# guilherme439/NuZero

Hardware: AMD Instinct MI355X
Metric: self-play games/sec (+ MCTS node-expansions/sec), Tic-Tac-Toe 100 sims/move (higher is better)
Workload: dtype f32; 1 GPU; Tic_Tac_Toe, 100 sims/move, 4096 concurrent self-play games per GPU (65536 games per round), RecurrentNet(2,1,64,2) 2 recurrent iterations f32, tree statistics f64, legacy TTT search config; concurrent_games_per_gpu=4096, games_per_round_per_gpu=65536, sims_per_move=100, parallelism=1 GPU

## Files before the change

### include/nuzero_amd.h

```cpp
#ifndef NUZERO_AMD_H
#define NUZERO_AMD_H

#include <stdint.h>

#ifdef __cplusplus
extern "C" {
#endif

typedef struct nz_engine nz_engine;
typedef struct nz_rng nz_rng;
typedef int nz_status;

enum {
  NZ_OK = 0,
  NZ_ERR_ARG = 1,
  NZ_ERR_HIP = 2,
  NZ_ERR_STATE = 3,
  NZ_ERR_OVERFLOW = 4
};

enum { NZ_GAME_TIC_TAC_TOE = 0 };
enum { NZ_ACT_TANH = 0, NZ_ACT_RELU = 1 };
enum { NZ_ARCH_RECURRENT = 0, NZ_ARCH_RESNET = 1, NZ_ARCH_CONVNET = 2 };

typedef struct nz_search_cfg {
  int32_t mcts_simulations;
  int32_t keep_subtree;
  double pb_c_base;
  double pb_c_init;
  int32_t number_of_softmax_moves;
  int32_t training;
  double epsilon_softmax_exploration;
  double epsilon_random_exploration;
  double value_factor;
  double root_exploration_fraction;
  double root_dist_alpha;
  double root_dist_beta;
} nz_search_cfg;

typedef struct nz_game_desc {
  int32_t game;
  int32_t negate_player;
} nz_game_desc;

typedef struct nz_net_desc {
  int32_t in_channels;
  int32_t policy_channels;
  int32_t width;
  int32_t num_blocks;
  int32_t recall;
  int32_t value_activation;
  int32_t arch;
  int32_t kernel_size;
  int32_t hex;
} nz_net_desc;

typedef struct nz_dims {
  int32_t n_games;
  int32_t n_slots;
  int32_t num_actions;
  int32_t max_moves;
  int32_t state_channels, rows, cols;
  int32_t node_capacity;
} nz_dims;

const char* nz_version(void);
const char* nz_last_error(const nz_engine* e);

nz_status nz_engine_create(nz_engine** out, const nz_search_cfg* cfg, const nz_game_desc* game,
                           int32_t n_games, int32_t device);
nz_status nz_engine_create_ex(nz_engine** out, const nz_search_cfg* cfg, const nz_game_desc* game,
                              int32_t n_slots, int32_t n_games, int32_t device);
void nz_engine_destroy(nz_engine* e);
nz_status nz_engine_dims(const nz_engine* e, nz_dims* out);

nz_status nz_engine_set_weights(nz_engine* e, const nz_net_desc* net, const float* const* weights,
                                int32_t n_tensors, int32_t recurrent_iterations);

nz_status nz_engine_set_table(nz_engine* e, const float* table, int32_t n_rows);

nz_status nz_engine_reset(nz_engine* e, void* stream);

nz_status nz_engine_root_children(nz_engine* e, int32_t* n_children_dev, void* stream);

nz_status nz_engine_move(nz_engine* e, const double* noise_dev, const double* uniforms_dev,
                         void* stream);

nz_status nz_engine_search(nz_engine* e, const double* noise_dev, void* stream);
nz_status nz_engine_apply(nz_engine* e, const int32_t* actions_dev, const double* uniforms_dev, void* stream);
nz_status nz_engine_last_actions(nz_engine* e, int32_t* actions_dev, void* stream);

nz_status nz_engine_alive(nz_engine* e, int32_t* alive_dev, void* stream);

nz_status nz_engine_live_games(nz_engine* e, int32_t* n_live_host, void* stream);

nz_status nz_engine_play(nz_engine* e, uint64_t base_seed, void* stream);
nz_status nz_engine_play_next(nz_engine* e, uint64_t base_seed, int32_t have_next, uint64_t next_base_seed, void* stream);

nz_status nz_engine_play_lockstep(nz_engine* e, uint64_t base_seed, void* stream);
nz_status nz_engine_desync_count(const nz_engine* e, int64_t* count_host);

nz_status nz_engine_export(nz_engine* e, float* states, int32_t* visits, int32_t* actions,
                           int32_t* lengths, int32_t* outcomes, int32_t* tree_size,
                           int32_t* n_children, double* bias, void* stream);

nz_status nz_engine_export_trace(nz_engine* e, double* child_prior, double* child_value_sum,
                                 double* root_value_sum, void* stream);

nz_status nz_engine_counters(nz_engine* e, int64_t* simulations_host, int64_t* expansions_host,
                             void* stream);
nz_status nz_engine_counters_ex(nz_engine* e, int64_t* out4_host, void* stream);
nz_status nz_engine_counters_n(nz_engine* e, int64_t* out_host, int32_t n_out, void* stream);

nz_status nz_engine_net_flops(const nz_engine* e, double* flops_host);
nz_status nz_engine_net_matrix_flops(const nz_engine* e, double* bf16_flops_host, double* f32_flops_host);

nz_status nz_net_forward(nz_engine* e, const float* states_dev, int32_t batch, float* logits_dev,
                         float* value_dev, float* probs_dev, void* stream);

nz_status nz_net_forward_stamps(nz_engine* e, const float* states_dev, int32_t batch, float* logits_dev,
                                float* value_dev, double* ticks4_host);

nz_status nz_engine_profile(nz_engine* e, int32_t enable);
nz_status nz_engine_profile_read(nz_engine* e, double* ms_host , int64_t* launches_host ,
                                 int64_t* net_positions_host);

nz_status nz_engine_phase_stamps(nz_engine* e, int32_t enable, double* out10_host);

typedef struct nz_scs nz_scs;
typedef struct nz_scs_desc {
  int32_t rows, cols, turns, stacking;
  const float* terrain;
  int32_t n_vp[2];
  const int32_t* vp;
  int32_t n_units;
  const int32_t* units;
  const uint8_t* arrival;
} nz_scs_desc;
nz_status nz_scs_create(nz_scs** out, const nz_scs_desc* desc, int32_t n_games, int32_t device);
void nz_scs_destroy(nz_scs* h);
const char* nz_scs_last_error(const nz_scs* h);
nz_status nz_scs_dims(const nz_scs* h, int32_t* planes, int32_t* rows, int32_t* cols, int32_t* channels);
nz_status nz_scs_reset(nz_scs* h, void* stream);
nz_status nz_scs_step(nz_scs* h, const int32_t* actions_dev, void* stream);
nz_status nz_scs_legal_mask(nz_scs* h, int8_t* mask_dev, void* stream);
nz_status nz_scs_state_image(nz_scs* h, float* image_dev, void* stream);
nz_status nz_scs_status(nz_scs* h, int32_t* status_dev, void* stream);

typedef struct nz_scs_search nz_scs_search;
nz_status nz_scs_search_create(nz_scs_search** out, const nz_scs_desc* desc, const nz_search_cfg* cfg,
                               int32_t n_games, int32_t nodes_per_game, int32_t device);
void nz_scs_search_destroy(nz_scs_search* h);
const char* nz_scs_search_last_error(const nz_scs_search* h);
nz_status nz_scs_search_reset(nz_scs_search* h, void* stream);
nz_status nz_scs_search_root_children(nz_scs_search* h, int32_t* n_children_dev, void* stream);
nz_status nz_scs_search_begin_move(nz_scs_search* h, const double* noise_dev, void* stream);
nz_status nz_scs_search_select(nz_scs_search* h, float* images_dev, int32_t* leaf_game_dev,
                               int32_t* n_leaves_host, void* stream);
nz_status nz_scs_search_expand(nz_scs_search* h, const float* probs_dev, const float* value_dev, void* stream);
nz_status nz_scs_search_end_move(nz_scs_search* h, const double* uniforms_dev, void* stream);
nz_status nz_scs_search_status(nz_scs_search* h, int32_t* status_dev, void* stream);
nz_status nz_scs_search_export(nz_scs_search* h, int32_t* actions, int32_t* tree_size, int32_t* n_children,
                               double* bias, double* root_value_sum, int32_t* child_action,
                               int32_t* child_visit, double* child_prior, double* child_value_sum,
                               int64_t* counters_host, void* stream);

typedef struct nz_boardnet nz_boardnet;
nz_status nz_boardnet_create(nz_boardnet** out, const nz_net_desc* net, int32_t rows, int32_t cols,
                             int32_t max_batch, int32_t device);
void nz_boardnet_destroy(nz_boardnet* h);
const char* nz_boardnet_last_error(const nz_boardnet* h);
nz_status nz_boardnet_set_weights(nz_boardnet* h, const float* const* weights, int32_t n_weights,
                                  int32_t recurrent_iterations);
nz_status nz_boardnet_forward(nz_boardnet* h, const float* images_dev, int32_t n, const int32_t* n_dev,
                              float* logits_dev, float* probs_dev, float* value_dev, void* stream);
nz_status nz_boardnet_input_rows(nz_boardnet* h, float** rows_dev, int32_t* row_stride);
nz_status nz_boardnet_forward_rows(nz_boardnet* h, int32_t n, const int32_t* n_dev, float* logits_dev, float* probs_dev,
                                   float* value_dev, void* stream);
int64_t nz_boardnet_flops(const nz_boardnet* h);
nz_status nz_boardnet_fused(nz_boardnet* h, int32_t enable, int32_t* available);
nz_status nz_boardnet_dims(const nz_boardnet* h, int32_t* in_channels, int32_t* policy_channels, int32_t* rows,
                           int32_t* cols, int32_t* max_batch);

nz_status nz_scs_search_play(nz_scs_search* h, nz_boardnet* net, const uint32_t* seeds_host, void* stream);
nz_status nz_scs_search_play_moves(nz_scs_search* h, nz_boardnet* net, const uint32_t* seeds_host, int32_t max_moves,
                                   void* stream);

nz_status nz_scs_search_play_round(nz_scs_search* h, nz_boardnet* net, const uint32_t* seeds_host, int64_t n_round,
                                   void* stream);
nz_status nz_scs_search_export_round(nz_scs_search* h, int32_t* actions, int32_t* tree_size, int32_t* n_children,
                                     double* bias, double* root_value_sum, int32_t* child_action, int32_t* child_visit,
                                     double* child_prior, double* child_value_sum, int32_t* status2,
                                     int64_t* counters_host, void* stream);
nz_status nz_scs_search_phase_ticks(nz_scs_search* h, int64_t* out6_host);
nz_status nz_scs_search_apply(nz_scs_search* h, const int32_t* actions_dev, const double* uniforms_dev, void* stream);
nz_status nz_scs_search_last_actions(nz_scs_search* h, int32_t* actions_dev, void* stream);

nz_status nz_scs_search_cache(nz_scs_search* h, int64_t max_entries);
nz_status nz_scs_search_cache_stats(nz_scs_search* h, int64_t* out4_host);
nz_status nz_scs_search_limits(const nz_scs_search* h, int32_t* max_moves, int32_t* max_children);
nz_status nz_scs_search_waves(const nz_scs_search* h, int64_t* waves);
nz_status nz_scs_search_persistent(nz_scs_search* h, int32_t enable, int32_t* used);
nz_status nz_scs_search_set_games(nz_scs_search* h, int64_t n, const float* terrain_host, const int32_t* vp_host,
                                  const uint32_t* mt_keys_host, const int32_t* mt_pos_host);
#define NZ_SCS_DRAW_MAP 1
#define NZ_SCS_DRAW_VP 2
typedef struct nz_scs_map_draw {
  int32_t n_types;
  const float* types;
  const double* cdf;
  int32_t order[2];
  int32_t number_vp[2];
  int32_t side_cols[4];
} nz_scs_map_draw;
nz_status nz_scs_search_set_map_draw(nz_scs_search* h, const nz_scs_map_draw* spec);
nz_status nz_scs_search_draw_games(nz_scs_search* h, int64_t n, const uint32_t* seeds_host, void* stream);
nz_status nz_scs_search_drawn_games(nz_scs_search* h, int64_t* n, float* terrain, int32_t* vp, uint32_t* mt_keys,
                                    int32_t* mt_pos, void* stream);
nz_status nz_scs_set_maps(nz_scs* h, const float* terrain_host, const int32_t* vp_host, void* stream);
nz_status nz_scs_search_persist_profile(nz_scs_search* h, int32_t enable, double* out4_host);
nz_status nz_scs_search_persist_ticks(nz_scs_search* h, int64_t* out13_host);
nz_status nz_scs_netbench(nz_boardnet* net, int32_t blocks, int32_t iters, uint64_t* ticks_host);
nz_status nz_boardnet_wide_stamps(uint64_t* out8);
nz_status nz_scs_search_record(nz_scs_search* h, const int32_t* games_host, int32_t n, int32_t capacity);
nz_status nz_scs_search_record_read(nz_scs_search* h, int32_t slot, int32_t* count, uint64_t* digests_host,
                                    float* probs_host, float* values_host);

typedef struct nz_scs_match_tally {
  int64_t matches, p1_wins, p2_wins, draws, unfinished, length_sum, length_max;
} nz_scs_match_tally;
nz_status nz_scs_match_play(nz_scs_search* a1, nz_boardnet* net1, nz_scs_search* a2, nz_boardnet* net2,
                            int32_t max_moves, void* stream);
nz_status nz_scs_match_result(nz_scs_search* a1, nz_scs_search* a2, nz_scs_match_tally* out_host, int32_t* actions_dev,
                              void* stream);

enum { NZ_AGENT_MCTS = 0, NZ_AGENT_POLICY = 1, NZ_AGENT_RANDOM = 2 };
typedef struct nz_scs_agent {
  int32_t kind;
  nz_boardnet* net;
  const uint32_t* seeds_host;
} nz_scs_agent;
nz_status nz_scs_agent_match_play(nz_scs_search* h, const nz_scs_agent* p1, const nz_scs_agent* p2, int32_t max_moves,
                                  void* stream);
nz_status nz_scs_agent_match_result(nz_scs_search* h, nz_scs_match_tally* out_host, int32_t* actions_dev, void* stream);
nz_status nz_scs_agent_match_decisions(nz_scs_search* h, int32_t side, int32_t* actions_dev, int32_t* n_legal_dev,
                                       float* probs_dev, void* stream);
nz_status nz_scs_agent_record(nz_scs_search* h, int32_t side, const int32_t* games_host, int32_t n, int32_t capacity);
nz_status nz_scs_agent_record_read(nz_scs_search* h, int32_t side, int32_t slot, int32_t* count, uint64_t* digests_host,
                                   float* probs_host, float* values_host);

nz_rng* nz_rng_create(uint32_t seed);
nz_rng* nz_rng_create_state(const uint32_t* key624, int32_t pos, int32_t has_gauss, double cached_gaussian);
nz_rng* nz_rng_clone(const nz_rng* r);
void nz_rng_destroy(nz_rng* r);
void nz_rng_seed(nz_rng* r, uint32_t seed);
uint32_t nz_rng_u32(nz_rng* r);
double nz_rng_double(nz_rng* r);
void nz_rng_gamma(nz_rng* r, double shape, double scale, int32_t n, double* out);

typedef struct nz_replay nz_replay;
nz_status nz_replay_create(nz_replay** out, int64_t capacity_positions, int32_t state_floats, int32_t num_actions,
                           int32_t device);
void nz_replay_destroy(nz_replay* h);
const char* nz_replay_last_error(const nz_replay* h);
nz_status nz_replay_dims(const nz_replay* h, int64_t* capacity, int32_t* state_floats, int32_t* num_actions);
nz_status nz_replay_append(nz_replay* h, const float* states_dev, const int32_t* visits_dev, const float* policies_dev,
                           const int32_t* child_action_dev, const int32_t* child_visit_dev, const int32_t* n_children_dev,
                           int32_t max_children, const int32_t* game_value_dev, int32_t rows_per_game,
                           const int64_t* dst_slot_dev, int64_t n_rows, int32_t game_index, void* stream);
nz_status nz_replay_gather(nz_replay* h, const int64_t* slots_dev, int64_t batch, float* states_out, float* policies_out,
                           float* values_out, int32_t* game_index_out, void* stream);
nz_status nz_replay_check(nz_replay* h, void* stream);

enum { NZ_LOSS_CE = 0, NZ_LOSS_KLD = 1, NZ_LOSS_MSE = 2 };
enum { NZ_LOSS_SE = 0, NZ_LOSS_AE = 1 };
nz_status nz_loss_forward_backward(const float* logits_dev, const float* values_dev, const float* target_policies_dev,
                                   const float* target_values_dev, int32_t batch, int32_t actions, int32_t policy_loss,
                                   int32_t value_loss, int32_t normalize_policy, float* losses3_dev, float* dlogits_dev,
                                   float* dvalues_dev, float* workspace_dev, void* stream);
const char* nz_loss_last_error(void);

#ifdef __cplusplus
}
#endif
#endif
```

### nuzero_amd/_lib.py

```python
import ctypes
import os

import torch

from ctypes import POINTER, Structure, c_char_p, c_double, c_int32, c_int64, c_uint32, c_uint64, c_void_p

_HERE = os.path.dirname(os.path.abspath(__file__))
LIB_PATH = os.environ.get("NZ_LIB_PATH") or os.path.join(_HERE, "csrc", "libnuzero_amd.so")

NZ_OK, NZ_ERR_ARG, NZ_ERR_HIP, NZ_ERR_STATE, NZ_ERR_OVERFLOW = range(5)
NZ_GAME_TIC_TAC_TOE = 0
NZ_ACT_TANH, NZ_ACT_RELU = 0, 1
NZ_ARCH_RECURRENT, NZ_ARCH_RESNET, NZ_ARCH_CONVNET = 0, 1, 2
NZ_LOSS_CE, NZ_LOSS_KLD, NZ_LOSS_MSE = 0, 1, 2
NZ_LOSS_SE, NZ_LOSS_AE = 0, 1


class SearchCfg(Structure):
    _fields_ = [("mcts_simulations", c_int32), ("keep_subtree", c_int32),
                ("pb_c_base", c_double), ("pb_c_init", c_double),
                ("number_of_softmax_moves", c_int32), ("training", c_int32),
                ("epsilon_softmax_exploration", c_double), ("epsilon_random_exploration", c_double),
                ("value_factor", c_double), ("root_exploration_fraction", c_double),
                ("root_dist_alpha", c_double), ("root_dist_beta", c_double)]


class GameDesc(Structure):
    _fields_ = [("game", c_int32), ("negate_player", c_int32)]


class NetDesc(Structure):
    _fields_ = [("in_channels", c_int32), ("policy_channels", c_int32), ("width", c_int32),
                ("num_blocks", c_int32), ("recall", c_int32), ("value_activation", c_int32),
                ("arch", c_int32), ("kernel_size", c_int32), ("hex", c_int32)]


class Dims(Structure):
    _fields_ = [("n_games", c_int32), ("n_slots", c_int32), ("num_actions", c_int32), ("max_moves", c_int32),
                ("state_channels", c_int32), ("rows", c_int32), ("cols", c_int32),
                ("node_capacity", c_int32)]


class ScsDesc(Structure):
    _fields_ = [("rows", c_int32), ("cols", c_int32), ("turns", c_int32), ("stacking", c_int32),
                ("terrain", c_void_p), ("n_vp", c_int32 * 2), ("vp", c_void_p), ("n_units", c_int32),
                ("units", c_void_p), ("arrival", c_void_p)]


NZ_SCS_DRAW_MAP, NZ_SCS_DRAW_VP = 1, 2


class ScsMapDraw(Structure):
    _fields_ = [("n_types", c_int32), ("types", c_void_p), ("cdf", c_void_p), ("order", c_int32 * 2),
                ("number_vp", c_int32 * 2), ("side_cols", c_int32 * 4)]


class ScsMatchTally(Structure):
    _fields_ = [(k, c_int64) for k in ("matches", "p1_wins", "p2_wins", "draws", "unfinished", "length_sum", "length_max")]


NZ_AGENT_MCTS, NZ_AGENT_POLICY, NZ_AGENT_RANDOM = 0, 1, 2


class ScsAgent(Structure):
    _fields_ = [("kind", c_int32), ("net", c_void_p), ("seeds_host", c_void_p)]


SIGNATURES = {
    "nz_version": (c_char_p, []),
    "nz_last_error": (c_char_p, [c_void_p]),
    "nz_engine_create": (c_int32, [POINTER(c_void_p), POINTER(SearchCfg), POINTER(GameDesc), c_int32, c_int32]),
    "nz_engine_create_ex": (c_int32, [POINTER(c_void_p), POINTER(SearchCfg), POINTER(GameDesc), c_int32, c_int32,
                                      c_int32]),
    "nz_engine_destroy": (None, [c_void_p]),
    "nz_engine_dims": (c_int32, [c_void_p, POINTER(Dims)]),
    "nz_engine_set_weights": (c_int32, [c_void_p, POINTER(NetDesc), POINTER(c_void_p), c_int32, c_int32]),
    "nz_engine_set_table": (c_int32, [c_void_p, c_void_p, c_int32]),
    "nz_engine_reset": (c_int32, [c_void_p, c_void_p]),
    "nz_engine_root_children": (c_int32, [c_void_p, c_void_p, c_void_p]),
    "nz_engine_search": (c_int32, [c_void_p, c_void_p, c_void_p]),
    "nz_engine_apply": (c_int32, [c_void_p, c_void_p, c_void_p, c_void_p]),
    "nz_engine_last_actions": (c_int32, [c_void_p, c_void_p, c_void_p]),
    "nz_engine_alive": (c_int32, [c_void_p, c_void_p, c_void_p]),
    "nz_engine_move": (c_int32, [c_void_p, c_void_p, c_void_p, c_void_p]),
    "nz_engine_live_games": (c_int32, [c_void_p, POINTER(c_int32), c_void_p]),
    "nz_engine_play": (c_int32, [c_void_p, c_uint64, c_void_p]),
    "nz_engine_play_next": (c_int32, [c_void_p, c_uint64, c_int32, c_uint64, c_void_p]),
    "nz_engine_play_lockstep": (c_int32, [c_void_p, c_uint64, c_void_p]),
    "nz_engine_desync_count": (c_int32, [c_void_p, POINTER(c_int64)]),
    "nz_engine_export": (c_int32, [c_void_p] + [c_void_p] * 8 + [c_void_p]),
    "nz_engine_export_trace": (c_int32, [c_void_p, c_void_p, c_void_p, c_void_p, c_void_p]),
    "nz_engine_counters": (c_int32, [c_void_p, POINTER(c_int64), POINTER(c_int64), c_void_p]),
    "nz_engine_counters_ex": (c_int32, [c_void_p, POINTER(c_int64), c_void_p]),
    "nz_engine_counters_n": (c_int32, [c_void_p, POINTER(c_int64), c_int32, c_void_p]),
    "nz_engine_net_flops": (c_int32, [c_void_p, POINTER(c_double)]),
    "nz_engine_net_matrix_flops": (c_int32, [c_void_p, POINTER(c_double), POINTER(c_double)]),
    "nz_net_forward": (c_int32, [c_void_p, c_void_p, c_int32, c_void_p, c_void_p, c_void_p, c_void_p]),
    "nz_net_forward_stamps": (c_int32, [c_void_p, c_void_p, c_int32, c_void_p, c_void_p, POINTER(c_double)]),
    "nz_engine_profile": (c_int32, [c_void_p, c_int32]),
    "nz_engine_profile_read": (c_int32, [c_void_p, POINTER(c_double), POINTER(c_int64), POINTER(c_int64)]),
    "nz_engine_phase_stamps": (c_int32, [c_void_p, c_int32, POINTER(c_double)]),
    "nz_scs_create": (c_int32, [POINTER(c_void_p), POINTER(ScsDesc), c_int32, c_int32]),
    "nz_scs_destroy": (None, [c_void_p]),
    "nz_scs_last_error": (c_char_p, [c_void_p]),
    "nz_scs_dims": (c_int32, [c_void_p, POINTER(c_int32), POINTER(c_int32), POINTER(c_int32), POINTER(c_int32)]),
    "nz_scs_reset": (c_int32, [c_void_p, c_void_p]),
    "nz_scs_step": (c_int32, [c_void_p, c_void_p, c_void_p]),
    "nz_scs_legal_mask": (c_int32, [c_void_p, c_void_p, c_void_p]),
    "nz_scs_state_image": (c_int32, [c_void_p, c_void_p, c_void_p]),
    "nz_scs_status": (c_int32, [c_void_p, c_void_p, c_void_p]),
    "nz_scs_search_create": (c_int32, [POINTER(c_void_p), POINTER(ScsDesc), POINTER(SearchCfg), c_int32, c_int32,
                                       c_int32]),
    "nz_scs_search_destroy": (None, [c_void_p]),
    "nz_scs_search_last_error": (c_char_p, [c_void_p]),
    "nz_scs_search_reset": (c_int32, [c_void_p, c_void_p]),
    "nz_scs_search_root_children": (c_int32, [c_void_p, c_void_p, c_void_p]),
    "nz_scs_search_begin_move": (c_int32, [c_void_p, c_void_p, c_void_p]),
    "nz_scs_search_select": (c_int32, [c_void_p, c_void_p, c_void_p, POINTER(c_int32), c_void_p]),
    "nz_scs_search_expand": (c_int32, [c_void_p, c_void_p, c_void_p, c_void_p]),
    "nz_scs_search_end_move": (c_int32, [c_void_p, c_void_p, c_void_p]),
    "nz_scs_search_status": (c_int32, [c_void_p, c_void_p, c_void_p]),
    "nz_scs_search_export": (c_int32, [c_void_p] + [c_void_p] * 9 + [POINTER(c_int64), c_void_p]),
    "nz_boardnet_create": (c_int32, [POINTER(c_void_p), POINTER(NetDesc), c_int32, c_int32, c_int32, c_int32]),
    "nz_boardnet_destroy": (None, [c_void_p]),
    "nz_boardnet_last_error": (c_char_p, [c_void_p]),
    "nz_boardnet_set_weights": (c_int32, [c_void_p, POINTER(c_void_p), c_int32, c_int32]),
    "nz_boardnet_forward": (c_int32, [c_void_p, c_void_p, c_int32, c_void_p, c_void_p, c_void_p, c_void_p, c_void_p]),
    "nz_boardnet_input_rows": (c_int32, [c_void_p, POINTER(c_void_p), POINTER(c_int32)]),
    "nz_boardnet_forward_rows": (c_int32, [c_void_p, c_int32, c_void_p, c_void_p, c_void_p, c_void_p, c_void_p]),
    "nz_boardnet_flops": (c_int64, [c_void_p]),
    "nz_boardnet_dims": (c_int32, [c_void_p] + [POINTER(c_int32)] * 5),
    "nz_boardnet_fused": (c_int32, [c_void_p, c_int32, POINTER(c_int32)]),
    "nz_scs_search_play": (c_int32, [c_void_p, c_void_p, c_void_p, c_void_p]),
    "nz_scs_search_play_moves": (c_int32, [c_void_p, c_void_p, c_void_p, c_int32, c_void_p]),
    "nz_scs_search_play_round": (c_int32, [c_void_p, c_void_p, c_void_p, c_int64, c_void_p]),
    "nz_scs_search_export_round": (c_int32, [c_void_p] + [c_void_p] * 10 + [c_void_p, c_void_p]),
    "nz_scs_search_waves": (c_int32, [c_void_p, POINTER(c_int64)]),
    "nz_scs_search_apply": (c_int32, [c_void_p, c_void_p, c_void_p, c_void_p]),
    "nz_scs_search_last_actions": (c_int32, [c_void_p, c_void_p, c_void_p]),
    "nz_scs_search_cache": (c_int32, [c_void_p, c_int64]),
    "nz_scs_search_cache_stats": (c_int32, [c_void_p, POINTER(c_int64)]),
    "nz_scs_search_limits": (c_int32, [c_void_p, POINTER(c_int32), POINTER(c_int32)]),
    "nz_scs_search_set_games": (c_int32, [c_void_p, c_int64, c_void_p, c_void_p, c_void_p, c_void_p]),
    "nz_scs_search_set_map_draw": (c_int32, [c_void_p, POINTER(ScsMapDraw)]),
    "nz_scs_search_draw_games": (c_int32, [c_void_p, c_int64, c_void_p, c_void_p]),
    "nz_scs_search_drawn_games": (c_int32, [c_void_p, POINTER(c_int64), c_void_p, c_void_p, c_void_p, c_void_p, c_void_p]),
    "nz_scs_set_maps": (c_int32, [c_void_p, c_void_p, c_void_p, c_void_p]),
    "nz_scs_search_persistent": (c_int32, [c_void_p, c_int32, POINTER(c_int32)]),
    "nz_scs_search_persist_ticks": (c_int32, [c_void_p, POINTER(c_int64)]),
    "nz_scs_search_persist_profile": (c_int32, [c_void_p, c_int32, POINTER(ctypes.c_double)]),
    "nz_scs_netbench": (c_int32, [c_void_p, c_int32, c_int32, c_void_p]),
    "nz_boardnet_wide_stamps": (c_int32, [c_void_p]),
    "nz_scs_search_record": (c_int32, [c_void_p, c_void_p, c_int32, c_int32]),
    "nz_scs_search_record_read": (c_int32, [c_void_p, c_int32, POINTER(c_int32), c_void_p, c_void_p, c_void_p]),
    "nz_scs_search_phase_ticks": (c_int32, [c_void_p, POINTER(c_int64)]),
    "nz_scs_match_play": (c_int32, [c_void_p, c_void_p, c_void_p, c_void_p, c_int32, c_void_p]),
    "nz_scs_match_result": (c_int32, [c_void_p, c_void_p, POINTER(ScsMatchTally), c_void_p, c_void_p]),
    "nz_scs_agent_match_play": (c_int32, [c_void_p, POINTER(ScsAgent), POINTER(ScsAgent), c_int32, c_void_p]),
    "nz_scs_agent_match_result": (c_int32, [c_void_p, POINTER(ScsMatchTally), c_void_p, c_void_p]),
    "nz_scs_agent_match_decisions": (c_int32, [c_void_p, c_int32, c_void_p, c_void_p, c_void_p, c_void_p]),
    "nz_scs_agent_record": (c_int32, [c_void_p, c_int32, c_void_p, c_int32, c_int32]),
    "nz_scs_agent_record_read": (c_int32, [c_void_p, c_int32, c_int32, POINTER(c_int32), c_void_p, c_void_p, c_void_p]),
    "nz_replay_create": (c_int32, [POINTER(c_void_p), c_int64, c_int32, c_int32, c_int32]),
    "nz_replay_destroy": (None, [c_void_p]),
    "nz_replay_last_error": (c_char_p, [c_void_p]),
    "nz_replay_dims": (c_int32, [c_void_p, POINTER(c_int64), POINTER(c_int32), POINTER(c_int32)]),
    "nz_replay_append": (c_int32, [c_void_p, c_void_p, c_void_p, c_void_p, c_void_p, c_void_p, c_void_p, c_int32,
                                   c_void_p, c_int32, c_void_p, c_int64, c_int32, c_void_p]),
    "nz_replay_gather": (c_int32, [c_void_p, c_void_p, c_int64, c_void_p, c_void_p, c_void_p, c_void_p, c_void_p]),
    "nz_replay_check": (c_int32, [c_void_p, c_void_p]),
    "nz_loss_forward_backward": (c_int32, [c_void_p, c_void_p, c_void_p, c_void_p, c_int32, c_int32, c_int32, c_int32,
                                           c_int32, c_void_p, c_void_p, c_void_p, c_void_p, c_void_p]),
    "nz_loss_last_error": (c_char_p, []),
    "nz_rng_create": (c_void_p, [c_uint32]),
    "nz_rng_create_state": (c_void_p, [c_void_p, c_int32, c_int32, c_double]),
    "nz_rng_clone": (c_void_p, [c_void_p]),
    "nz_rng_destroy": (None, [c_void_p]),
    "nz_rng_seed": (None, [c_void_p, c_uint32]),
    "nz_rng_u32": (c_uint32, [c_void_p]),
    "nz_rng_double": (c_double, [c_void_p]),
    "nz_rng_gamma": (None, [c_void_p, c_double, c_double, c_int32, POINTER(c_double)]),
}


def _load():
    if not os.path.exists(LIB_PATH):
        raise ImportError(
            f"{LIB_PATH} is missing: build it with `python -m nuzero_amd.build` "
            "(the engine has no CPU or PyTorch fallback)")
    lib = ctypes.CDLL(LIB_PATH)
    for name, (res, args) in SIGNATURES.items():
        fn = getattr(lib, name)
        fn.restype = res
        fn.argtypes = args
    return lib


lib = _load()


class NzError(RuntimeError):
    def __init__(self, code, message):
        super().__init__(f"nuzero_amd error {code}: {message}")
        self.code = code


def check(status, handle=None):
    if status != NZ_OK:
        msg = lib.nz_last_error(handle)
        raise NzError(status, msg.decode() if msg else "")
```

### nuzero_amd/csrc/engine.h

```cpp
#pragma once
#include <hip/hip_runtime.h>
#include <stdint.h>

#include "../../include/nuzero_amd.h"

namespace nz {

constexpr int TTT_ACTIONS = 9;
constexpr int TTT_MAX_MOVES = 9;
constexpr int TTT_TABLE_ROWS = 19683;
constexpr int MAX_PATH = 16;
constexpr int LANES_PER_GAME = 16;

constexpr uint32_t TO_PLAY_UNSET = 15u;
__host__ __device__ inline uint32_t pack_meta(uint32_t n_children, uint32_t action, uint32_t to_play,
                                              uint32_t term) {
  return n_children | (action << 12) | (to_play << 24) | (term << 28);
}
__host__ __device__ inline uint32_t meta_children(uint32_t m) { return m & 0xfffu; }
__host__ __device__ inline uint32_t meta_action(uint32_t m) { return (m >> 12) & 0xfffu; }
__host__ __device__ inline uint32_t meta_to_play(uint32_t m) { return (m >> 24) & 0xfu; }

struct __attribute__((aligned(16))) TNode {
  double value_sum;
  double q;
  double prior;
  int32_t visit;
  uint32_t first;
  uint32_t meta;
  uint32_t pad[3];
};
static_assert(sizeof(TNode) == 48, "three 16-byte loads per node");

struct TreeParams {
  TNode* nodes;
  int32_t cap;
  int32_t n_games;
  int32_t n_slots;
  int32_t* next_game;
  uint32_t* board;
  int32_t* length;
  int32_t* alive;
  int32_t* outcome;
  int32_t* root;
  int32_t* node_count;
  int32_t* sims_left;
  int32_t* pending;
  uint32_t* leaf_board;
  int32_t* path;
  int32_t* path_len;
  int32_t* sim_count;
  int32_t* exp_count;
  int32_t* sel_nodes;
  int32_t* sel_children;
  int32_t* new_nodes;
  int32_t* n_root_children;
  int32_t* desync;
  int32_t* leaf_count;
  uint32_t* leaf_boards;
  const float* leaf_logits;
  const float* leaf_value;
  const float* table;
  const double* bias_tab;
  const double* sqrt_tab;
  int32_t tab_len;
  int32_t sims;
  int32_t negate_player;
  double value_factor;
  double frac, one_minus_frac;
  int32_t training;
  int32_t softmax_moves;
  double eps_softmax, eps_random;
  int32_t sims_per_cycle;
  int32_t slots_per_wg;
  int32_t max_cycles;
  int32_t* error_flag;
  uint32_t* hist_board;
  int32_t* hist_action;
  int32_t* hist_visits;
  int32_t* hist_tree_size;
  int32_t* hist_children;
  double* hist_bias;
  double* hist_prior;
  double* hist_value_sum;
  double* hist_root_value_sum;
};

void launch_reset(const TreeParams& p, hipStream_t s);
void launch_noise(const TreeParams& p, const double* noise, hipStream_t s);
void launch_advance(const TreeParams& p, int iteration, hipStream_t s);
void launch_finish_move(const TreeParams& p, const double* uniforms, const int32_t* forced, hipStream_t s);
void launch_last_actions(const TreeParams& p, int32_t* actions, hipStream_t s);
void launch_export_states(const TreeParams& p, float* states, hipStream_t s);
void launch_export_visits(const TreeParams& p, int32_t* visits, int32_t* actions, int32_t* tree_size,
                          int32_t* n_children, double* bias, hipStream_t s);

int selfplay_blocks(int n_slots, int slots_per_wg);
void launch_selfplay(const TreeParams& p, const struct NetProgram* prog_dev, int n_layers, const float* weights,
                     const double* noise, const double* uniforms, unsigned long long* stamps, hipStream_t s);

constexpr int NET_KG_CHANNELS = 32;
constexpr int NET_KG_DWORDS = 9 * 3 * 64 * 4;
constexpr int NET_ACT_BUFFERS = 2;
constexpr int NET_DST_POLICY = NET_ACT_BUFFERS;
constexpr int NET_DST_VALUE = NET_ACT_BUFFERS + 1;
constexpr int NET_DST_STRIP = NET_ACT_BUFFERS + 2;
constexpr int NET_SSLOT_SPLIT = -1;

struct NetJob {
  int32_t w_off;
  int32_t wx_off;
  int32_t next_w_off;
  int8_t kgroups;
  int8_t sslot;
  int16_t nt;
  int8_t extra;
  int8_t og;
  int8_t src, dst;
  int8_t res;
  int8_t act;
  int8_t stage_end;
  int8_t dtile;
};
constexpr int NET_WAVES_HOST = 8;
constexpr int NET_MAX_JOBS = 192;
constexpr int OG_NONE = 7;
struct NetProgram {
  int32_t n_jobs[NET_WAVES_HOST];
  int32_t first_w_off[NET_WAVES_HOST];
  NetJob jobs[NET_WAVES_HOST][NET_MAX_JOBS];
};

void launch_net(const NetProgram* prog_dev, int n_layers, const float* packed_weights,
                const uint32_t* boards, const float* states, const int32_t* count_dev, int max_positions,
                float* logits, float* value, float* probs, unsigned long long* stamps, hipStream_t s);

}
```

### nuzero_amd/csrc/engine.hip

```cpp
#include <cmath>
#include <cstdarg>
#include <cstdio>
#include <cstdlib>
#include <cstring>
#include <algorithm>
#include <string>
#include <thread>
#include <vector>

#include "engine.h"
#include "hip_own.hpp"

using namespace nz;

namespace {
thread_local std::string g_create_error;

struct ProfileSpan {
  Event a, b;
  int cls = 0;
};

struct EngineArrays {
  DevBuf<TNode> nodes;
  DevBuf<uint32_t> board, leaf_board, leaf_boards, hist_board;
  DevBuf<int32_t> next_game, length, alive, outcome, root, node_count, sims_left, pending, path, path_len, sim_count, exp_count,
      sel_nodes, sel_children, new_nodes, n_root_children, desync, leaf_count, error_flag, hist_action, hist_visits,
      hist_tree_size, hist_children;
  DevBuf<float> leaf_logits, leaf_value;
  DevBuf<double> bias_tab, sqrt_tab, hist_bias, hist_prior, hist_value_sum, hist_root_value_sum;
  DevBuf<double> noise, uniforms, game_noise, game_uniforms;
  DevBuf<unsigned long long> stamps;
  DevBuf<NetProgram> prog;
};
}

struct nz_engine {
  nz_search_cfg cfg;
  nz_game_desc game;
  int device = 0;
  int n_games = 0;
  int n_slots = 0;
  int cap = 0;
  int tab_len = 0;
  TreeParams tp;
  EngineArrays dev;
  std::string error;
  bool have_net = false, have_table = false;
  nz_net_desc net;
  int iters = 0;
  NetProgram prog_host;
  DevBuf<float> weights_dev, table_dev;
  const float* borrowed_weights = nullptr;
  double executed_bf16_flops_per_position = 0.0, executed_f32_flops_per_position = 0.0;
  double algorithmic_flops_per_position = 0.0;
  PinnedBuf<int32_t> h_children, h_alive, h_desync;
  PinnedBuf<double> h_noise, h_uniforms;
  std::vector<nz_rng*> rngs;
  PinnedBuf<double> h_game_noise, h_game_uniforms;
  PinnedBuf<double> h_next_noise, h_next_uniforms;
  bool next_ready = false;
  uint64_t next_seed = 0;
  nz_engine* fallback = nullptr;
  int64_t desync_total = 0;
  bool stamps = false;
  bool profile = false;
  std::vector<ProfileSpan> spans;
  int64_t net_positions = 0;
};

namespace {

nz_status fail(nz_engine* e, nz_status code, const char* fmt, ...) {
  char buf[512];
  va_list ap;
  va_start(ap, fmt);
  vsnprintf(buf, sizeof(buf), fmt, ap);
  va_end(ap);
  if (e) e->error = buf;
  else g_create_error = buf;
  return code;
}

#define NZ_HIP(e, call)                                                                          \
  do {                                                                                           \
    hipError_t err__ = (call);                                                                   \
    if (err__ != hipSuccess)                                                                     \
      return fail((e), NZ_ERR_HIP, "%s failed: %s (%s:%d)", #call, hipGetErrorString(err__), __FILE__, __LINE__); \
  } while (0)

const float* net_weights(const nz_engine* e) { return e->borrowed_weights ? e->borrowed_weights : e->weights_dev.get(); }

struct Span {
  nz_engine* e;
  hipStream_t s;
  ProfileSpan sp{};
  bool on;
  Span(nz_engine* e_, hipStream_t s_, int cls) : e(e_), s(s_), on(e_->profile) {
    if (!on) return;
    sp.cls = cls;
    if (!sp.a.create() || !sp.b.create()) { on = false; return; }
    (void)hipEventRecord(sp.a.get(), s);
  }
  ~Span() {
    if (!on) return;
    (void)hipEventRecord(sp.b.get(), s);
    e->spans.push_back(std::move(sp));
  }
};

int head_channel(int width, int out, int n_layers, int idx) {
  const double step = (double)(out - width) / n_layers;
  double prev = width;
  int c = width;
  for (int i = 0; i < idx; ++i) {
    prev += step;
    c = (int)prev;
  }
  return c;
}

struct PackedConv {
  int cout, cin, cin_main, kgroups, ntiles, extra;
  int32_t w_off, wx_off;
};
static void split3(float a, uint16_t p[3]) {
  float r = a;
  for (int i = 0; i < 3; ++i) {
    uint32_t bits;
    memcpy(&bits, &r, 4);
    bits &= 0xFFFF0000u;
    p[i] = (uint16_t)(bits >> 16);
    float t;
    memcpy(&t, &bits, 4);
    r = r - t;
  }
}
PackedConv pack_conv(const float* w, int cout, int cin, int cin_main, std::vector<float>& out) {
  PackedConv pc{};
  pc.cout = cout; pc.cin = cin; pc.cin_main = cin_main;
  pc.ntiles = (cout + 15) / 16;
  pc.kgroups = (cin_main + NET_KG_CHANNELS - 1) / NET_KG_CHANNELS;
  pc.extra = cin > cin_main ? 1 : 0;
  while (out.size() % 4) out.push_back(0.f);
  pc.w_off = (int32_t)out.size();
  auto weight = [&](int co, int ci, int t) { return co < cout && ci < cin_main ? w[((size_t)co * cin + ci) * 9 + t] : 0.f; };
  for (int nt = 0; nt < pc.ntiles; ++nt)
    for (int kg = 0; kg < pc.kgroups; ++kg)
      for (int t = 0; t < 9; ++t)
        for (int piece = 0; piece < 3; ++piece)
          for (int lane = 0; lane < 64; ++lane)
            for (int pr = 0; pr < 4; ++pr) {
              uint16_t lo[3], hi[3];
              const int co = nt * 16 + (lane & 15), ci = kg * 32 + (lane >> 4) * 8 + 2 * pr;
              split3(weight(co, ci, t), lo);
              split3(weight(co, ci + 1, t), hi);
              const uint32_t word = (uint32_t)lo[piece] | ((uint32_t)hi[piece] << 16);
              float f;
              memcpy(&f, &word, 4);
              out.push_back(f);
            }
  pc.wx_off = (int32_t)out.size();
  if (pc.extra)
    for (int nt = 0; nt < pc.ntiles; ++nt)
      for (int t = 0; t < 9; ++t)
        for (int lane = 0; lane < 64; ++lane) {
          const int co = nt * 16 + (lane & 15);
          const int ci = cin_main + (lane >> 4);
          out.push_back(co < cout && ci < cin ? w[((size_t)co * cin + ci) * 9 + t] : 0.f);
        }
  return pc;
}

struct StageConv {
  int tensor, src, dst, res, act;
  bool split;
  int sslot = 0;
  int dtile = 0;
};
const int og_taps[7] = {49, 13, 12, 12, 12, 26, 23};
const int JOB_OVERHEAD = 12;
bool add_stage(NetProgram& pg, const std::vector<PackedConv>& convs, const std::vector<StageConv>& stage) {
  struct Unit { NetJob job; int cost; };
  struct Tile { const StageConv* sc; int nt; };
  std::vector<Tile> tiles;
  for (const StageConv& sc : stage) {
    const PackedConv& pc = convs[sc.tensor];
    if (!sc.split || pc.ntiles >= NET_WAVES_HOST) return false;
    for (int nt = 0; nt < pc.ntiles; ++nt) tiles.push_back({&sc, nt});
  }
  auto make_units = [&](unsigned quarters, std::vector<Unit>& units) {
    units.clear();
    for (size_t t = 0; t < tiles.size(); ++t) {
      const StageConv& sc = *tiles[t].sc;
      const PackedConv& pc = convs[sc.tensor];
      const int nt = tiles[t].nt;
      const bool q = (quarters >> t) & 1;
      for (int og = q ? 1 : 5; og <= (q ? 4 : 6); ++og) {
        NetJob j{};
        j.w_off = pc.w_off + nt * pc.kgroups * NET_KG_DWORDS;
        j.wx_off = pc.wx_off + nt * 9 * 64;
        j.kgroups = (int8_t)pc.kgroups;
        j.sslot = (int8_t)sc.sslot;
        j.nt = (int16_t)nt;
        j.extra = (int8_t)pc.extra;
        j.og = (int8_t)og;
        j.src = (int8_t)sc.src; j.dst = (int8_t)sc.dst; j.res = (int8_t)sc.res; j.act = (int8_t)sc.act;
        j.dtile = (int8_t)(sc.dtile + nt);
        if (sc.dst < NET_ACT_BUFFERS && j.dtile >= 4) { j.dst = NET_DST_STRIP; j.dtile = (int8_t)(j.dtile - 4); }
        units.push_back({j, og_taps[og] * (3 * pc.kgroups + pc.extra) + JOB_OVERHEAD});
      }
    }
    std::stable_sort(units.begin(), units.end(), [](const Unit& a, const Unit& b) { return a.cost > b.cost; });
  };
  auto deal = [](const std::vector<Unit>& units, int (&load)[NET_WAVES_HOST], int* who) {
    for (int w = 0; w < NET_WAVES_HOST; ++w) load[w] = 0;
    for (size_t u = 0; u < units.size(); ++u) {
      int w = 0;
      for (int i = 1; i < NET_WAVES_HOST; ++i)
        if (load[i] < load[w]) w = i;
      load[w] += units[u].cost;
      if (who) who[u] = w;
    }
  };
  unsigned best = 2 * tiles.size() >= (size_t)NET_WAVES_HOST ? 0u : (1u << tiles.size()) - 1u;
  std::vector<Unit> units;
  if (stage.size() > 1) {
    long best_key = -1;
    for (unsigned m = 0; m < (1u << tiles.size()); ++m) {
      int load[NET_WAVES_HOST];
      make_units(m, units);
      deal(units, load, nullptr);
      int simd = 0, wave = 0;
      for (int w = 0; w < NET_WAVES_HOST; ++w) wave = std::max(wave, load[w]);
      for (int w = 0; w < NET_WAVES_HOST / 2; ++w) simd = std::max(simd, load[w] + load[w + NET_WAVES_HOST / 2]);
      const long key = (long)simd * 65536 + wave;
      if (best_key < 0 || key < best_key) { best_key = key; best = m; }
    }
  }
  make_units(best, units);
  for (const Unit& u : units) {
    if (u.job.dst == NET_DST_STRIP && (u.job.dtile != 0 || u.job.act != 1 || u.job.res >= 0)) return false;
    if (u.job.sslot == NET_SSLOT_SPLIT && u.job.kgroups != 1) return false;
  }
  int load[NET_WAVES_HOST];
  std::vector<int> who(units.size());
  deal(units, load, who.data());
  int first[NET_WAVES_HOST];
  for (int w = 0; w < NET_WAVES_HOST; ++w) first[w] = pg.n_jobs[w];
  for (size_t u = 0; u < units.size(); ++u) {
    const int w = who[u];
    if (pg.n_jobs[w] >= NET_MAX_JOBS) return false;
    pg.jobs[w][pg.n_jobs[w]++] = units[u].job;
  }
  for (int w = 0; w < NET_WAVES_HOST; ++w) {
    if (pg.n_jobs[w] == first[w]) {
      if (pg.n_jobs[w] >= NET_MAX_JOBS) return false;
      NetJob j{};
      j.og = OG_NONE;
      pg.jobs[w][pg.n_jobs[w]++] = j;
    }
    pg.jobs[w][pg.n_jobs[w] - 1].stage_end = 1;
  }
  return true;
}

hipStream_t as_stream(void* s) { return static_cast<hipStream_t>(s); }

nz_status check_device_flag(nz_engine* e, hipStream_t s) {
  int32_t flag = 0;
  NZ_HIP(e, hipMemcpyAsync(&flag, e->tp.error_flag, sizeof(flag), hipMemcpyDeviceToHost, s));
  NZ_HIP(e, hipStreamSynchronize(s));
  if (flag != 0)
    return fail(e, NZ_ERR_OVERFLOW, "device check failed (flag %d: 1 = tree arena full, 2 = visit table too short, "
                                    "4 = move finished before its search, 8 = forced action is not legal, "
                                    "64 = persistent kernel gave up after its cycle bound)", flag);
  return NZ_OK;
}

}

extern "C" {

const char* nz_version(void) { return "nuzero_amd 0.1 (gfx950)"; }

const char* nz_last_error(const nz_engine* e) { return e ? e->error.c_str() : g_create_error.c_str(); }

nz_status nz_engine_create(nz_engine** out, const nz_search_cfg* cfg, const nz_game_desc* game, int32_t n_games,
                           int32_t device) {
  return nz_engine_create_ex(out, cfg, game, n_games, n_games, device);
}

nz_status nz_engine_create_ex(nz_engine** out, const nz_search_cfg* cfg, const nz_game_desc* game, int32_t n_slots,
                              int32_t n_games, int32_t device) {
  if (!out || !cfg || !game) return fail(nullptr, NZ_ERR_ARG, "null argument");
  if (n_slots <= 0) return fail(nullptr, NZ_ERR_ARG, "n_slots must be positive");
  if (n_slots > n_games) n_slots = n_games > 0 ? n_games : n_slots;
  *out = nullptr;
  if (game->game != NZ_GAME_TIC_TAC_TOE) return fail(nullptr, NZ_ERR_ARG, "unsupported game %d", game->game);
  if (n_games <= 0) return fail(nullptr, NZ_ERR_ARG, "n_games must be positive");
  if (cfg->mcts_simulations <= 0) return fail(nullptr, NZ_ERR_ARG, "mcts_simulations must be positive");
  if (!cfg->keep_subtree)
    return fail(nullptr, NZ_ERR_ARG, "keep_subtree = False is not supported: the reference never resets the root "
                                     "in that mode (Training/Gamer.py:78-79) and every shipped config sets True");
  if (!(cfg->pb_c_base > 0)) return fail(nullptr, NZ_ERR_ARG, "pb_c_base must be positive");
  int n_dev = 0;
  if (hipGetDeviceCount(&n_dev) != hipSuccess || n_dev <= 0)
    return fail(nullptr, NZ_ERR_HIP, "no HIP device available (the engine has no CPU fallback)");
  if (device < 0 || device >= n_dev) return fail(nullptr, NZ_ERR_ARG, "device %d out of range", device);

  nz_engine* e = new nz_engine;
  e->cfg = *cfg;
  e->game = *game;
  e->device = device;
  e->n_games = n_games;
  e->n_slots = n_slots;
  e->cap = 1 + cfg->mcts_simulations * 45;
  e->tab_len = cfg->mcts_simulations * TTT_MAX_MOVES + 2;
  auto bail = [&](nz_status s) {
    g_create_error = e->error;
    nz_engine_destroy(e);
    return s;
  };
  if (hipSetDevice(device) != hipSuccess) return bail(fail(e, NZ_ERR_HIP, "hipSetDevice(%d) failed", device));

  TreeParams& p = e->tp;
  memset(&p, 0, sizeof(p));
  const size_t G = n_games, N = (size_t)n_slots * (size_t)e->cap, GT = G * TTT_MAX_MOVES, GTA = GT * TTT_ACTIONS;
#define P(f, n)                                                                           \
  if (!e->dev.f.ensure(n)) return bail(fail(e, NZ_ERR_HIP, "device allocation failed")); \
  p.f = e->dev.f.get()
  P(nodes, N);
  P(board, G); P(length, G); P(alive, G); P(outcome, G); P(root, G); P(node_count, G);
  P(sims_left, G); P(pending, G); P(leaf_board, G); P(path, G * MAX_PATH); P(path_len, G);
  P(sim_count, G); P(exp_count, G); P(sel_nodes, G); P(sel_children, G); P(new_nodes, G); P(desync, G); P(n_root_children, G);
  P(leaf_count, 2); P(leaf_boards, G); P(leaf_logits, G * TTT_ACTIONS); P(leaf_value, G);
  P(error_flag, 1);
  P(hist_board, GT); P(hist_action, GT); P(hist_visits, GTA); P(hist_tree_size, GT);
  P(hist_children, GT); P(hist_bias, GT); P(hist_prior, GTA); P(hist_value_sum, GTA);
  P(hist_root_value_sum, GT);
  P(bias_tab, e->tab_len); P(sqrt_tab, e->tab_len);
  P(next_game, 1);
#undef P
  EngineArrays& d = e->dev;
  if (!d.noise.ensure(G * TTT_ACTIONS) || !d.uniforms.ensure(G * 3) || !d.game_noise.ensure(GTA) ||
      !d.game_uniforms.ensure(GT * 3) || !d.stamps.ensure((size_t)n_slots * 6) ||
      !d.prog.ensure(1))
    return bail(fail(e, NZ_ERR_HIP, "device allocation failed"));
  p.cap = e->cap;
  p.n_games = n_games;
  p.n_slots = n_slots;
  p.table = nullptr;
  p.tab_len = e->tab_len;
  p.sims = cfg->mcts_simulations;
  p.negate_player = game->negate_player;
  p.value_factor = cfg->value_factor;
  p.frac = cfg->root_exploration_fraction;
  p.one_minus_frac = 1.0 - cfg->root_exploration_fraction;
  p.training = cfg->training;
  p.softmax_moves = cfg->number_of_softmax_moves;
  p.eps_softmax = cfg->epsilon_softmax_exploration;
  p.eps_random = cfg->epsilon_random_exploration;
  {
    hipDeviceProp_t prop;
    int n_cu = 256;
    if (hipGetDeviceProperties(&prop, e->device) == hipSuccess && prop.multiProcessorCount > 0) n_cu = prop.multiProcessorCount;
    p.slots_per_wg = std::min(16, std::max(1, (n_slots + n_cu - 1) / n_cu));
    if (const char* v = getenv("NZ_SLOTS_PER_WG")) p.slots_per_wg = std::min(16, std::max(1, atoi(v)));
  }
  p.sims_per_cycle = 16;
  if (const char* v = getenv("NZ_SIMS_PER_CYCLE")) p.sims_per_cycle = std::max(1, atoi(v));
  {
    const double games_per_slot = std::ceil((double)p.n_games / (double)p.n_slots) + 2.0;
    const double bound = 16.0 * games_per_slot * TTT_MAX_MOVES * ((double)cfg->mcts_simulations + 2.0);
    p.max_cycles = (int32_t)std::min(bound, 2.0e9);
  }

  std::vector<double> hb(e->tab_len), hs(e->tab_len);
  for (int n = 0; n < e->tab_len; ++n) {
    hb[n] = std::log(((double)n + cfg->pb_c_base + 1.0) / cfg->pb_c_base) + cfg->pb_c_init;
    hs[n] = std::sqrt((double)n);
  }
  if (hipMemcpy(d.bias_tab.get(), hb.data(), hb.size() * sizeof(double), hipMemcpyHostToDevice) != hipSuccess ||
      hipMemcpy(d.sqrt_tab.get(), hs.data(), hs.size() * sizeof(double), hipMemcpyHostToDevice) != hipSuccess)
    return bail(fail(e, NZ_ERR_HIP, "table upload failed"));

  if (!e->h_children.ensure(G) || !e->h_alive.ensure(G) || !e->h_noise.ensure(G * TTT_ACTIONS) || !e->h_uniforms.ensure(G * 3) ||
      !e->h_game_noise.ensure(GTA) || !e->h_game_uniforms.ensure(GT * 3) || !e->h_next_noise.ensure(GTA) ||
      !e->h_next_uniforms.ensure(GT * 3) || !e->h_desync.ensure(G))
    return bail(fail(e, NZ_ERR_HIP, "pinned host allocation failed"));
  for (PinnedBuf<double>* b : {&e->h_noise, &e->h_uniforms, &e->h_game_noise, &e->h_game_uniforms, &e->h_next_noise, &e->h_next_uniforms})
    memset(b->get(), 0, b->size() * sizeof(double));

  launch_reset(p, nullptr);
  if (hipDeviceSynchronize() != hipSuccess) return bail(fail(e, NZ_ERR_HIP, "reset kernel failed"));
  *out = e;
  return NZ_OK;
}

void nz_engine_destroy(nz_engine* e) {
  if (!e) return;
  (void)hipSetDevice(e->device);
  (void)hipDeviceSynchronize();
  if (e->fallback) nz_engine_destroy(e->fallback);
  for (nz_rng* r : e->rngs) nz_rng_destroy(r);
  delete e;
}

nz_status nz_engine_dims(const nz_engine* e, nz_dims* out) {
  if (!e || !out) return NZ_ERR_ARG;
  out->n_games = e->n_games;
  out->n_slots = e->n_slots;
  out->num_actions = TTT_ACTIONS;
  out->max_moves = TTT_MAX_MOVES;
  out->state_channels = 2;
  out->rows = 3;
  out->cols = 3;
  out->node_capacity = e->cap;
  return NZ_OK;
}

nz_status nz_engine_set_weights(nz_engine* e, const nz_net_desc* net, const float* const* weights,
                                int32_t n_tensors, int32_t recurrent_iterations) {
  if (!e || !net || !weights) return NZ_ERR_ARG;
  if (net->hex) return fail(e, NZ_ERR_ARG, "hexagonal convolutions are built for nz_boardnet_* only");
  if (net->in_channels != 2 || net->policy_channels != 1)
    return fail(e, NZ_ERR_ARG, "Tic-Tac-Toe nets take 2 input planes and 1 policy plane");
  if (net->width <= 0 || net->width > 64 || net->width % 4 != 0)
    return fail(e, NZ_ERR_ARG, "width must be a multiple of 4 in (0, 64]");
  if (net->num_blocks < 0 || recurrent_iterations < 0) return fail(e, NZ_ERR_ARG, "negative block/iteration count");
  const int arch = net->arch;
  if (arch != NZ_ARCH_RECURRENT && arch != NZ_ARCH_RESNET && arch != NZ_ARCH_CONVNET)
    return fail(e, NZ_ERR_ARG, "unknown architecture %d", arch);
  const int trunk_k = arch == NZ_ARCH_CONVNET ? net->kernel_size : 3;
  if (trunk_k != 1 && trunk_k != 3) return fail(e, NZ_ERR_ARG, "ConvNet kernel_size must be 1 or 3");
  const bool recall = arch == NZ_ARCH_RECURRENT && net->recall;
  const int iterations = arch == NZ_ARCH_RECURRENT ? recurrent_iterations : 1;
  const int trunk_tensors = arch == NZ_ARCH_CONVNET ? 1 + net->num_blocks : 1 + (recall ? 1 : 0) + 2 * net->num_blocks;
  const int expect = trunk_tensors + 2 + 4;
  if (n_tensors != expect) return fail(e, NZ_ERR_ARG, "expected %d weight tensors, got %d", expect, n_tensors);
  if (1 + iterations * (trunk_tensors - 1) + 24 > NET_MAX_JOBS)
    return fail(e, NZ_ERR_ARG, "too many layers for one fused launch (%d iterations)", recurrent_iterations);
  NZ_HIP(e, hipSetDevice(e->device));

  const int W = net->width, IN = net->in_channels;
  struct Shape { int cout, cin, k; };
  std::vector<Shape> shapes;
  shapes.push_back({W, IN, trunk_k});
  if (recall) shapes.push_back({W, W + IN, 3});
  for (int i = (int)shapes.size(); i < trunk_tensors; ++i) shapes.push_back({W, W, trunk_k});
  for (int i = 0; i < 2; ++i)
    shapes.push_back({head_channel(W, net->policy_channels, 2, i + 1), head_channel(W, net->policy_channels, 2, i), 3});
  for (int i = 0; i < 4; ++i) shapes.push_back({head_channel(W, 1, 4, i + 1), head_channel(W, 1, 4, i), 3});

  std::vector<std::vector<float>> host(n_tensors);
  for (int i = 0; i < n_tensors; ++i) {
    const size_t n_in = (size_t)shapes[i].cout * shapes[i].cin * shapes[i].k * shapes[i].k;
    std::vector<float> raw(n_in);
    NZ_HIP(e, hipMemcpy(raw.data(), weights[i], n_in * sizeof(float), hipMemcpyDefault));
    if (shapes[i].k == 3) {
      host[i].swap(raw);
    } else {
      host[i].assign((size_t)shapes[i].cout * shapes[i].cin * 9, 0.f);
      for (size_t j = 0; j < n_in; ++j) host[i][j * 9 + 4] = raw[j];
    }
  }

  std::vector<float> packed;
  std::vector<PackedConv> convs(n_tensors);
  double flops = 0.0;
  for (int i = 0; i < n_tensors; ++i) {
    const bool with_planes = (i == 0) || (recall && i == 1);
    const int cin_main = with_planes ? shapes[i].cin - IN : shapes[i].cin;
    convs[i] = pack_conv(host[i].data(), shapes[i].cout, shapes[i].cin, cin_main, packed);
  }

  NetProgram& pg = e->prog_host;
  memset(&pg, 0, sizeof(pg));
  bool ok = true;
  int cur = 0;
  auto stage = [&](std::vector<StageConv> convs_in_stage) {
    for (const StageConv& sc : convs_in_stage)
      flops += 2.0 * shapes[sc.tensor].cout * shapes[sc.tensor].cin * (shapes[sc.tensor].k == 3 ? 49.0 : 9.0);
    ok = ok && add_stage(pg, convs, convs_in_stage);
  };
  if (arch == NZ_ARCH_CONVNET) {
    stage({{0, 0, cur, -1, 3, true}});
    for (int i = 1; i < trunk_tensors; ++i) { stage({{i, cur, cur ^ 1, -1, 3, true}}); cur ^= 1; }
  } else {
    stage({{0, 0, cur, -1, 1, true}});
    const int first_block = recall ? 2 : 1;
    for (int it = 0; it < iterations; ++it) {
      if (recall) { stage({{1, cur, cur ^ 1, -1, 0, true}}); cur ^= 1; }
      for (int b = 0; b < net->num_blocks; ++b) {
        stage({{first_block + 2 * b, cur, cur ^ 1, -1, 1, true}});
        stage({{first_block + 2 * b + 1, cur ^ 1, cur, cur, 1, true}});
      }
    }
  }
  const int ph = trunk_tensors, vh = ph + 2;
  const int vact = net->value_activation == NZ_ACT_RELU ? 1 : 2;
  const int side = cur ^ 1;
  const int tv0 = convs[vh].ntiles, tp0 = convs[ph].ntiles;
  if (tv0 + tp0 > 5 || (tv0 + tp0 == 5 && tv0 != 3)) return fail(e, NZ_ERR_ARG, "head layout: %d + %d tiles", tv0, tp0);
  const int p1_sslot = tv0 + tp0 <= 4 ? 2 * tv0 : NET_SSLOT_SPLIT;
  stage({{vh, cur, side, -1, vact, true, 0, 0}, {ph, cur, side, -1, 1, true, 0, tv0}});
  stage({{vh + 1, side, cur, -1, vact, true}, {ph + 1, side, NET_DST_POLICY, -1, 0, true, p1_sslot, 0}});
  stage({{vh + 2, cur, side, -1, vact, true}});
  stage({{vh + 3, side, NET_DST_VALUE, -1, 0, true}});
  if (!ok) return fail(e, NZ_ERR_ARG, "network too deep for one fused launch (%d iterations)", recurrent_iterations);
  for (int w = 0; w < NET_WAVES_HOST; ++w) {
    int32_t next = -1;
    for (int j = pg.n_jobs[w] - 1; j >= 0; --j) {
      pg.jobs[w][j].next_w_off = next;
      if (pg.jobs[w][j].og != OG_NONE && pg.jobs[w][j].kgroups > 0) next = pg.jobs[w][j].w_off;
    }
    pg.first_w_off[w] = next;
  }
  e->algorithmic_flops_per_position = flops;
  {
    double bf16 = 0.0, f32 = 0.0;
    for (int w = 0; w < NET_WAVES_HOST; ++w)
      for (int j = 0; j < pg.n_jobs[w]; ++j) {
        const NetJob& job = pg.jobs[w][j];
        if (job.og == OG_NONE) continue;
        bf16 += (double)og_taps[job.og] * job.kgroups * 6.0 * (2.0 * 16 * 16 * 32);
        f32 += (double)og_taps[job.og] * job.extra * (2.0 * 16 * 16 * 4);
      }
    e->executed_bf16_flops_per_position = bf16 / 16.0;
    e->executed_f32_flops_per_position = f32 / 16.0;
  }

  if (!e->weights_dev.ensure(packed.size())) return fail(e, NZ_ERR_HIP, "device allocation failed (%zu packed weights)", packed.size());
  NZ_HIP(e, hipMemcpy(e->weights_dev.get(), packed.data(), packed.size() * sizeof(float), hipMemcpyHostToDevice));
  NZ_HIP(e, hipMemcpy(e->dev.prog.get(), &pg, sizeof(pg), hipMemcpyHostToDevice));
  e->net = *net;
  e->iters = recurrent_iterations;
  e->have_net = true;
  e->have_table = false;
  e->tp.table = nullptr;
  return NZ_OK;
}

nz_status nz_engine_set_table(nz_engine* e, const float* table, int32_t n_rows) {
  if (!e || !table) return NZ_ERR_ARG;
  if (n_rows != TTT_TABLE_ROWS) return fail(e, NZ_ERR_ARG, "table must have %d rows", TTT_TABLE_ROWS);
  NZ_HIP(e, hipSetDevice(e->device));
  if (!e->table_dev.ensure((size_t)TTT_TABLE_ROWS * 10)) return fail(e, NZ_ERR_HIP, "device allocation failed (table)");
  NZ_HIP(e, hipMemcpy(e->table_dev.get(), table, (size_t)TTT_TABLE_ROWS * 10 * sizeof(float), hipMemcpyDefault));
  e->tp.table = e->table_dev.get();
  e->have_table = true;
  return NZ_OK;
}

nz_status nz_engine_reset(nz_engine* e, void* stream) {
  if (!e) return NZ_ERR_ARG;
  NZ_HIP(e, hipSetDevice(e->device));
  Span sp(e, as_stream(stream), 2);
  launch_reset(e->tp, as_stream(stream));
  NZ_HIP(e, hipGetLastError());
  return NZ_OK;
}

nz_status nz_engine_root_children(nz_engine* e, int32_t* n_children_dev, void* stream) {
  if (!e || !n_children_dev) return NZ_ERR_ARG;
  NZ_HIP(e, hipMemcpyAsync(n_children_dev, e->tp.n_root_children, e->n_games * sizeof(int32_t),
                           hipMemcpyDeviceToDevice, as_stream(stream)));
  return NZ_OK;
}

nz_status nz_engine_alive(nz_engine* e, int32_t* alive_dev, void* stream) {
  if (!e || !alive_dev) return NZ_ERR_ARG;
  NZ_HIP(e, hipMemcpyAsync(alive_dev, e->tp.alive, e->n_games * sizeof(int32_t), hipMemcpyDeviceToDevice,
                           as_stream(stream)));
  return NZ_OK;
}

static nz_status search_lockstep(nz_engine* e, const double* noise_dev, hipStream_t s) {
  const TreeParams& p = e->tp;
  if (e->cfg.training) {
    Span sp(e, s, 2);
    launch_noise(p, noise_dev, s);
  }
  if (p.table != nullptr) {
    Span sp(e, s, 0);
    launch_advance(p, 0, s);
  } else {
    const int sims = e->cfg.mcts_simulations;
    for (int it = 0; it <= sims; ++it) {
      {
        Span sp(e, s, 0);
        launch_advance(p, it, s);
      }
      if (it == sims) break;
      {
        Span sp(e, s, 1);
        launch_net(e->dev.prog.get(), 0, net_weights(e), p.leaf_boards, nullptr,
                   p.leaf_count + (it & 1), e->n_games, e->dev.leaf_logits.get(), e->dev.leaf_value.get(), nullptr, nullptr, s);
      }
    }
  }
  return NZ_OK;
}

static nz_status check_lockstep_call(nz_engine* e, const double* noise_dev, const double* uniforms_dev, bool need_uni) {
  if (e->n_slots != e->n_games)
    return fail(e, NZ_ERR_STATE, "the lock-step route needs n_slots == n_games (every game of the round in flight)");
  if (!e->have_net && !e->have_table) return fail(e, NZ_ERR_STATE, "no network: call nz_engine_set_weights first");
  if (e->cfg.training && (!noise_dev || (need_uni && !uniforms_dev)))
    return fail(e, NZ_ERR_ARG, "training search needs noise and uniforms");
  return NZ_OK;
}

nz_status nz_engine_move(nz_engine* e, const double* noise_dev, const double* uniforms_dev, void* stream) {
  if (!e) return NZ_ERR_ARG;
  nz_status st = check_lockstep_call(e, noise_dev, uniforms_dev, true);
  if (st != NZ_OK) return st;
  NZ_HIP(e, hipSetDevice(e->device));
  hipStream_t s = as_stream(stream);
  search_lockstep(e, noise_dev, s);
  {
    Span sp(e, s, 2);
    launch_finish_move(e->tp, uniforms_dev, nullptr, s);
  }
  NZ_HIP(e, hipGetLastError());
  return NZ_OK;
}

nz_status nz_engine_search(nz_engine* e, const double* noise_dev, void* stream) {
  if (!e) return NZ_ERR_ARG;
  nz_status st = check_lockstep_call(e, noise_dev, nullptr, false);
  if (st != NZ_OK) return st;
  NZ_HIP(e, hipSetDevice(e->device));
  search_lockstep(e, noise_dev, as_stream(stream));
  NZ_HIP(e, hipGetLastError());
  return NZ_OK;
}

nz_status nz_engine_apply(nz_engine* e, const int32_t* actions_dev, const double* uniforms_dev, void* stream) {
  if (!e) return NZ_ERR_ARG;
  if (e->n_slots != e->n_games)
    return fail(e, NZ_ERR_STATE, "the lock-step route needs n_slots == n_games (every game of the round in flight)");
  if (!actions_dev && e->cfg.training && !uniforms_dev)
    return fail(e, NZ_ERR_ARG, "a training engine choosing its own action needs uniforms");
  NZ_HIP(e, hipSetDevice(e->device));
  hipStream_t s = as_stream(stream);
  {
    Span sp(e, s, 2);
    launch_finish_move(e->tp, uniforms_dev, actions_dev, s);
  }
  NZ_HIP(e, hipGetLastError());
  return NZ_OK;
}

nz_status nz_engine_last_actions(nz_engine* e, int32_t* actions_dev, void* stream) {
  if (!e || !actions_dev) return NZ_ERR_ARG;
  NZ_HIP(e, hipSetDevice(e->device));
  launch_last_actions(e->tp, actions_dev, as_stream(stream));
  NZ_HIP(e, hipGetLastError());
  return NZ_OK;
}

nz_status nz_engine_live_games(nz_engine* e, int32_t* n_live_host, void* stream) {
  if (!e || !n_live_host) return NZ_ERR_ARG;
  hipStream_t s = as_stream(stream);
  NZ_HIP(e, hipMemcpyAsync(e->h_alive.get(), e->tp.alive, e->n_games * sizeof(int32_t), hipMemcpyDeviceToHost, s));
  NZ_HIP(e, hipStreamSynchronize(s));
  int n = 0;
  for (int g = 0; g < e->n_games; ++g) n += e->h_alive[g] != 0;
  *n_live_host = n;
  return check_device_flag(e, s);
}

static void draw_move(nz_rng* r, const nz_search_cfg& c, int move, int n_children, double* noise9, double* uni3) {
  nz_rng_gamma(r, c.root_dist_alpha, c.root_dist_beta, n_children, noise9);
  double u1 = 0.0, u2 = 0.0, u3 = 0.0;
  bool choice;
  if (move < c.number_of_softmax_moves) {
    choice = true;
  } else {
    u1 = nz_rng_double(r);
    u2 = nz_rng_double(r);
    choice = (u1 < c.epsilon_softmax_exploration) || (u2 < c.epsilon_random_exploration);
  }
  if (choice) u3 = nz_rng_double(r);
  uni3[0] = u1;
  uni3[1] = u2;
  uni3[2] = u3;
}

static void ensure_rngs(nz_engine* e) {
  if ((int)e->rngs.size() == e->n_games) return;
  for (nz_rng* r : e->rngs) nz_rng_destroy(r);
  e->rngs.assign(e->n_games, nullptr);
  for (int g = 0; g < e->n_games; ++g) e->rngs[g] = nz_rng_create(0);
}

static nz_status play_lockstep(nz_engine* e, const uint32_t* seeds, void* stream) {
  if (e->n_slots != e->n_games)
    return fail(e, NZ_ERR_STATE, "the lock-step route needs n_slots == n_games (every game of the round in flight)");
  hipStream_t s = as_stream(stream);
  const int G = e->n_games;
  const nz_search_cfg& c = e->cfg;
  if (c.training) {
    ensure_rngs(e);
    for (int g = 0; g < G; ++g) nz_rng_seed(e->rngs[g], seeds[g]);
  }
  nz_status st = nz_engine_reset(e, stream);
  if (st != NZ_OK) return st;
  for (int move = 0; move < TTT_MAX_MOVES; ++move) {
    NZ_HIP(e, hipMemcpyAsync(e->h_children.get(), e->tp.n_root_children, G * sizeof(int32_t), hipMemcpyDeviceToHost, s));
    NZ_HIP(e, hipMemcpyAsync(e->h_alive.get(), e->tp.alive, G * sizeof(int32_t), hipMemcpyDeviceToHost, s));
    NZ_HIP(e, hipStreamSynchronize(s));
    int live = 0;
    for (int g = 0; g < G; ++g) live += e->h_alive[g] != 0;
    if (live == 0) break;
    if (c.training) {
      for (int g = 0; g < G; ++g)
        if (e->h_alive[g])
          draw_move(e->rngs[g], c, move, e->h_children[g], e->h_noise.get() + (size_t)g * TTT_ACTIONS, e->h_uniforms.get() + g * 3);
      NZ_HIP(e, hipMemcpyAsync(e->dev.noise.get(), e->h_noise.get(), (size_t)G * TTT_ACTIONS * sizeof(double), hipMemcpyHostToDevice, s));
      NZ_HIP(e, hipMemcpyAsync(e->dev.uniforms.get(), e->h_uniforms.get(), (size_t)G * 3 * sizeof(double), hipMemcpyHostToDevice, s));
    }
    st = nz_engine_move(e, e->dev.noise.get(), e->dev.uniforms.get(), stream);
    if (st != NZ_OK) return st;
  }
  return check_device_flag(e, s);
}

nz_status nz_engine_play_lockstep(nz_engine* e, uint64_t base_seed, void* stream) {
  if (!e) return NZ_ERR_ARG;
  if (!e->have_net && !e->have_table) return fail(e, NZ_ERR_STATE, "no network: call nz_engine_set_weights first");
  NZ_HIP(e, hipSetDevice(e->device));
  std::vector<uint32_t> seeds(e->n_games);
  for (int g = 0; g < e->n_games; ++g) seeds[g] = (uint32_t)((base_seed + (uint64_t)g) & 0xffffffffu);
  return play_lockstep(e, seeds.data(), stream);
}

static nz_status replay_desynced(nz_engine* e, const std::vector<int>& games, uint64_t base_seed, void* stream) {
  hipStream_t s = as_stream(stream);
  const int n = (int)games.size();
  if (e->fallback && e->fallback->n_games < n) {
    nz_engine_destroy(e->fallback);
    e->fallback = nullptr;
  }
  if (!e->fallback) {
    nz_engine* f = nullptr;
    nz_status st = nz_engine_create(&f, &e->cfg, &e->game, std::max(n, 16), e->device);
    if (st != NZ_OK) return fail(e, st, "fallback engine: %s", nz_last_error(nullptr));
    e->fallback = f;
  }
  nz_engine* f = e->fallback;
  f->borrowed_weights = e->weights_dev.get();
  f->tp.table = e->tp.table;
  f->have_net = e->have_net;
  f->have_table = e->have_table;
  f->prog_host = e->prog_host;
  NZ_HIP(e, hipMemcpy(f->dev.prog.get(), &e->prog_host, sizeof(NetProgram), hipMemcpyHostToDevice));
  std::vector<uint32_t> seeds(f->n_games, 0u);
  for (int i = 0; i < n; ++i) seeds[i] = (uint32_t)((base_seed + (uint64_t)games[i]) & 0xffffffffu);
  nz_status st = play_lockstep(f, seeds.data(), stream);
  if (st != NZ_OK) return fail(e, st, "fallback replay: %s", f->error.c_str());
  const TreeParams &a = f->tp, &b = e->tp;
  for (int i = 0; i < n; ++i) {
    const size_t g = games[i];
#define ROW(field, per_game)                                                                               \
  NZ_HIP(e, hipMemcpyAsync(b.field + g * (per_game), a.field + (size_t)i * (per_game),                     \
                           (per_game) * sizeof(*a.field), hipMemcpyDeviceToDevice, s))
    ROW(hist_board, TTT_MAX_MOVES); ROW(hist_action, TTT_MAX_MOVES); ROW(hist_tree_size, TTT_MAX_MOVES);
    ROW(hist_children, TTT_MAX_MOVES); ROW(hist_bias, TTT_MAX_MOVES); ROW(hist_root_value_sum, TTT_MAX_MOVES);
    ROW(hist_visits, TTT_MAX_MOVES * TTT_ACTIONS); ROW(hist_prior, TTT_MAX_MOVES * TTT_ACTIONS);
    ROW(hist_value_sum, TTT_MAX_MOVES * TTT_ACTIONS);
    ROW(length, 1); ROW(outcome, 1); ROW(board, 1);
    ROW(sim_count, 1); ROW(exp_count, 1); ROW(sel_nodes, 1); ROW(sel_children, 1); ROW(new_nodes, 1);
#undef ROW
  }
  NZ_HIP(e, hipStreamSynchronize(s));
  return NZ_OK;
}

static void draw_round(nz_engine* e, uint64_t base_seed, double* noise, double* uniforms) {
  const int G = e->n_games;
  const nz_search_cfg& c = e->cfg;
  const int n_threads = std::max(1, std::min(16, (int)std::thread::hardware_concurrency()));
  auto work = [&](int t) {
    for (int g = t; g < G; g += n_threads) {
      nz_rng* r = e->rngs[g];
      nz_rng_seed(r, (uint32_t)((base_seed + (uint64_t)g) & 0xffffffffu));
      for (int m = 0; m < TTT_MAX_MOVES; ++m)
        draw_move(r, c, m, m == 0 ? 0 : TTT_ACTIONS - m, noise + ((size_t)g * TTT_MAX_MOVES + m) * TTT_ACTIONS,
                  uniforms + ((size_t)g * TTT_MAX_MOVES + m) * 3);
    }
  };
  if (G < 256 || n_threads == 1) {
    for (int t = 0; t < n_threads; ++t) work(t);
  } else {
    std::vector<std::thread> pool;
    for (int t = 0; t < n_threads; ++t) pool.emplace_back(work, t);
    for (auto& th : pool) th.join();
  }
}

nz_status nz_engine_play(nz_engine* e, uint64_t base_seed, void* stream) {
  return nz_engine_play_next(e, base_seed, 0, 0, stream);
}

nz_status nz_engine_play_next(nz_engine* e, uint64_t base_seed, int32_t have_next, uint64_t next_base_seed, void* stream) {
  if (!e) return NZ_ERR_ARG;
  if (!e->have_net && !e->have_table) return fail(e, NZ_ERR_STATE, "no network: call nz_engine_set_weights first");
  NZ_HIP(e, hipSetDevice(e->device));
  hipStream_t s = as_stream(stream);
  const int G = e->n_games;
  const nz_search_cfg& c = e->cfg;

  nz_status st = nz_engine_reset(e, stream);
  if (st != NZ_OK) return st;
  if (c.training) {
    ensure_rngs(e);
    const size_t GT = (size_t)G * TTT_MAX_MOVES;
    if (e->next_ready && e->next_seed == base_seed) {
      std::swap(e->h_game_noise, e->h_next_noise);
      std::swap(e->h_game_uniforms, e->h_next_uniforms);
    } else {
      draw_round(e, base_seed, e->h_game_noise.get(), e->h_game_uniforms.get());
    }
    e->next_ready = false;
    NZ_HIP(e, hipMemcpyAsync(e->dev.game_noise.get(), e->h_game_noise.get(), GT * TTT_ACTIONS * sizeof(double), hipMemcpyHostToDevice, s));
    NZ_HIP(e, hipMemcpyAsync(e->dev.game_uniforms.get(), e->h_game_uniforms.get(), GT * 3 * sizeof(double), hipMemcpyHostToDevice, s));
  }
  {
    Span sp(e, s, 0);
    launch_selfplay(e->tp, e->dev.prog.get(), 0, net_weights(e),
                    c.training ? e->dev.game_noise.get() : nullptr, c.training ? e->dev.game_uniforms.get() : nullptr,
                    e->stamps ? e->dev.stamps.get() : nullptr, s);
  }
  NZ_HIP(e, hipGetLastError());
  if (c.training && have_next) {
    draw_round(e, next_base_seed, e->h_next_noise.get(), e->h_next_uniforms.get());
    e->next_ready = true;
    e->next_seed = next_base_seed;
  }
  st = check_device_flag(e, s);
  if (st != NZ_OK) return st;
  if (c.training) {
    NZ_HIP(e, hipMemcpyAsync(e->h_desync.get(), e->tp.desync, G * sizeof(int32_t), hipMemcpyDeviceToHost, s));
    NZ_HIP(e, hipStreamSynchronize(s));
    std::vector<int> bad;
    for (int g = 0; g < G; ++g)
      if (e->h_desync[g]) bad.push_back(g);
    if (!bad.empty()) {
      e->desync_total += (int64_t)bad.size();
      st = replay_desynced(e, bad, base_seed, stream);
      if (st != NZ_OK) return st;
    }
  }
  return NZ_OK;
}

nz_status nz_engine_phase_stamps(nz_engine* e, int32_t enable, double* out4_host) {
  if (!e) return NZ_ERR_ARG;
  if (out4_host) {
    const int blocks = selfplay_blocks(e->n_slots, e->tp.slots_per_wg);
    std::vector<unsigned long long> h((size_t)blocks * 6);
    NZ_HIP(e, hipSetDevice(e->device));
    NZ_HIP(e, hipDeviceSynchronize());
    NZ_HIP(e, hipMemcpy(h.data(), e->dev.stamps.get(), h.size() * sizeof(unsigned long long), hipMemcpyDeviceToHost));
    double sum[4] = {0, 0, 0, 0};
    double max_total = 0;
    for (int b = 0; b < blocks; ++b) {
      for (int i = 0; i < 4; ++i) sum[i] += (double)h[b * 4 + i];
      max_total = std::max(max_total, (double)h[b * 4 + 3]);
    }
    out4_host[0] = sum[0] / blocks;
    out4_host[1] = sum[1] / std::max(sum[3], 1.0);
    out4_host[2] = sum[2] / std::max(sum[3], 1.0);
    out4_host[3] = sum[3] / blocks / std::max(max_total, 1.0);
    out4_host[4] = sum[2] / std::max(sum[0], 1.0);
    out4_host[5] = sum[1] / std::max(sum[0], 1.0);
    out4_host[6] = max_total;
    out4_host[7] = (double)blocks;
    double fin = 0, exp = 0;
    for (int b = 0; b < blocks; ++b) {
      fin += (double)h[(size_t)blocks * 4 + b * 2];
      exp += (double)h[(size_t)blocks * 4 + b * 2 + 1];
    }
    out4_host[8] = fin / std::max(sum[0], 1.0);
    out4_host[9] = exp / std::max(sum[0], 1.0);
  }
  e->stamps = enable != 0;
  return NZ_OK;
}

nz_status nz_engine_desync_count(const nz_engine* e, int64_t* count_host) {
  if (!e || !count_host) return NZ_ERR_ARG;
  *count_host = e->desync_total;
  return NZ_OK;
}

nz_status nz_engine_export(nz_engine* e, float* states, int32_t* visits, int32_t* actions, int32_t* lengths,
                           int32_t* outcomes, int32_t* tree_size, int32_t* n_children, double* bias, void* stream) {
  if (!e) return NZ_ERR_ARG;
  NZ_HIP(e, hipSetDevice(e->device));
  hipStream_t s = as_stream(stream);
  Span sp(e, s, 2);
  if (states) launch_export_states(e->tp, states, s);
  if (visits || actions || tree_size || n_children || bias)
    launch_export_visits(e->tp, visits, actions, tree_size, n_children, bias, s);
  if (lengths)
    NZ_HIP(e, hipMemcpyAsync(lengths, e->tp.length, e->n_games * sizeof(int32_t), hipMemcpyDeviceToDevice, s));
  if (outcomes)
    NZ_HIP(e, hipMemcpyAsync(outcomes, e->tp.outcome, e->n_games * sizeof(int32_t), hipMemcpyDeviceToDevice, s));
  NZ_HIP(e, hipGetLastError());
  return NZ_OK;
}

nz_status nz_engine_export_trace(nz_engine* e, double* child_prior, double* child_value_sum, double* root_value_sum,
                                 void* stream) {
  if (!e) return NZ_ERR_ARG;
  hipStream_t s = as_stream(stream);
  const size_t GT = (size_t)e->n_games * TTT_MAX_MOVES;
  if (child_prior)
    NZ_HIP(e, hipMemcpyAsync(child_prior, e->tp.hist_prior, GT * TTT_ACTIONS * sizeof(double), hipMemcpyDeviceToDevice, s));
  if (child_value_sum)
    NZ_HIP(e, hipMemcpyAsync(child_value_sum, e->tp.hist_value_sum, GT * TTT_ACTIONS * sizeof(double), hipMemcpyDeviceToDevice, s));
  if (root_value_sum)
    NZ_HIP(e, hipMemcpyAsync(root_value_sum, e->tp.hist_root_value_sum, GT * sizeof(double), hipMemcpyDeviceToDevice, s));
  return NZ_OK;
}

nz_status nz_engine_counters(nz_engine* e, int64_t* simulations_host, int64_t* expansions_host, void* stream) {
  if (!e) return NZ_ERR_ARG;
  hipStream_t s = as_stream(stream);
  std::vector<int32_t> a(e->n_games), b(e->n_games);
  NZ_HIP(e, hipMemcpyAsync(a.data(), e->tp.sim_count, a.size() * sizeof(int32_t), hipMemcpyDeviceToHost, s));
  NZ_HIP(e, hipMemcpyAsync(b.data(), e->tp.exp_count, b.size() * sizeof(int32_t), hipMemcpyDeviceToHost, s));
  NZ_HIP(e, hipStreamSynchronize(s));
  int64_t sa = 0, sb = 0;
  for (int g = 0; g < e->n_games; ++g) { sa += a[g]; sb += b[g]; }
  if (simulations_host) *simulations_host = sa;
  if (expansions_host) *expansions_host = sb;
  return NZ_OK;
}

nz_status nz_engine_counters_n(nz_engine* e, int64_t* out_host, int32_t n_out, void* stream) {
  if (!e || !out_host || n_out < 1 || n_out > 5) return NZ_ERR_ARG;
  hipStream_t s = as_stream(stream);
  const int32_t* src[5] = {e->tp.sim_count, e->tp.exp_count, e->tp.sel_nodes, e->tp.sel_children, e->tp.new_nodes};
  std::vector<int32_t> h(e->n_games);
  for (int i = 0; i < n_out; ++i) {
    NZ_HIP(e, hipMemcpyAsync(h.data(), src[i], h.size() * sizeof(int32_t), hipMemcpyDeviceToHost, s));
    NZ_HIP(e, hipStreamSynchronize(s));
    int64_t sum = 0;
    for (int32_t v : h) sum += v;
    out_host[i] = sum;
  }
  return NZ_OK;
}

nz_status nz_engine_counters_ex(nz_engine* e, int64_t* out4_host, void* stream) {
  return nz_engine_counters_n(e, out4_host, 4, stream);
}

nz_status nz_engine_net_flops(const nz_engine* e, double* flops_host) {
  if (!e || !flops_host) return NZ_ERR_ARG;
  *flops_host = e->algorithmic_flops_per_position;
  return NZ_OK;
}

nz_status nz_engine_net_matrix_flops(const nz_engine* e, double* bf16_flops_host, double* f32_flops_host) {
  if (!e || !bf16_flops_host || !f32_flops_host) return NZ_ERR_ARG;
  *bf16_flops_host = e->executed_bf16_flops_per_position;
  *f32_flops_host = e->executed_f32_flops_per_position;
  return NZ_OK;
}

nz_status nz_net_forward(nz_engine* e, const float* states_dev, int32_t batch, float* logits_dev, float* value_dev,
                         float* probs_dev, void* stream) {
  if (!e || !states_dev || !logits_dev || !value_dev) return NZ_ERR_ARG;
  if (!e->have_net) return fail(e, NZ_ERR_STATE, "no network: call nz_engine_set_weights first");
  if (batch <= 0) return NZ_OK;
  NZ_HIP(e, hipSetDevice(e->device));
  Span sp(e, as_stream(stream), 1);
  launch_net(e->dev.prog.get(), 0, net_weights(e), nullptr, states_dev, nullptr, batch, logits_dev,
             value_dev, probs_dev, nullptr, as_stream(stream));
  NZ_HIP(e, hipGetLastError());
  return NZ_OK;
}

nz_status nz_net_forward_stamps(nz_engine* e, const float* states_dev, int32_t batch, float* logits_dev,
                                float* value_dev, double* ticks4_host) {
  if (!e || !states_dev || !logits_dev || !value_dev || !ticks4_host) return NZ_ERR_ARG;
  if (!e->have_net) return fail(e, NZ_ERR_STATE, "no network: call nz_engine_set_weights first");
  NZ_HIP(e, hipSetDevice(e->device));
  const int blocks = (batch + 15) / 16;
  DevBuf<unsigned long long> stamps;
  if (!stamps.ensure((size_t)blocks * 4)) return fail(e, NZ_ERR_HIP, "device allocation failed");
  launch_net(e->dev.prog.get(), 0, net_weights(e), nullptr, states_dev, nullptr, batch, logits_dev, value_dev, nullptr, stamps.get(),
             nullptr);
  std::vector<unsigned long long> h((size_t)blocks * 4);
  hipError_t err = hipMemcpy(h.data(), stamps.get(), h.size() * sizeof(unsigned long long), hipMemcpyDeviceToHost);
  if (err != hipSuccess) return fail(e, NZ_ERR_HIP, "stamp read-back failed: %s", hipGetErrorString(err));
  for (int i = 0; i < 4; ++i) {
    double sum = 0;
    for (int b = 0; b < blocks; ++b) sum += (double)h[(size_t)b * 4 + i];
    ticks4_host[i] = sum / blocks;
  }
  return NZ_OK;
}

nz_status nz_engine_profile(nz_engine* e, int32_t enable) {
  if (!e) return NZ_ERR_ARG;
  e->spans.clear();
  e->profile = enable != 0;
  return NZ_OK;
}

nz_status nz_engine_profile_read(nz_engine* e, double* ms_host, int64_t* launches_host, int64_t* net_positions_host) {
  if (!e) return NZ_ERR_ARG;
  NZ_HIP(e, hipSetDevice(e->device));
  NZ_HIP(e, hipDeviceSynchronize());
  double ms[3] = {0, 0, 0};
  int64_t n[3] = {0, 0, 0};
  for (auto& sp : e->spans) {
    float t = 0.f;
    NZ_HIP(e, hipEventElapsedTime(&t, sp.a.get(), sp.b.get()));
    ms[sp.cls] += t;
    n[sp.cls] += 1;
  }
  for (int i = 0; i < 3; ++i) {
    if (ms_host) ms_host[i] = ms[i];
    if (launches_host) launches_host[i] = n[i];
  }
  if (net_positions_host) *net_positions_host = 0;
  return NZ_OK;
}

}
```

### nuzero_amd/csrc/net_dev.hpp

```cpp
#pragma once
#include "engine.h"

namespace nz {

typedef float f32x4 __attribute__((ext_vector_type(4)));
typedef __bf16 bf16x8 __attribute__((ext_vector_type(8)));
typedef uint32_t u32x4 __attribute__((ext_vector_type(4)));
typedef uint32_t u32x2 __attribute__((ext_vector_type(2)));

constexpr int POS = 16;
constexpr int CELLS = 9;
constexpr int ROW = 64;
constexpr int NET_WAVES = 8;
constexpr int NET_THREADS = NET_WAVES * 64;
constexpr int NET_BUFFERS = NET_ACT_BUFFERS;
constexpr int PIECE_BYTES = CELLS * POS * ROW * 2;
constexpr int ACT_BYTES = 3 * PIECE_BYTES;
constexpr int ACT_FLOATS = ACT_BYTES / 4;
constexpr int INP_FLOATS = CELLS * POS * 4;
constexpr int VAL_FLOATS = CELLS * POS;
constexpr int STRIP_PIECE_BYTES = CELLS * POS * 16 * 2;
constexpr int STRIP_FLOATS = 3 * STRIP_PIECE_BYTES / 4;
constexpr int NET_LDS_FLOATS = NET_BUFFERS * ACT_FLOATS + INP_FLOATS + VAL_FLOATS + STRIP_FLOATS;
constexpr int TAP_DWORDS = 3 * 64 * 4;
constexpr int W_RING = 3;
static_assert(NET_WAVES == NET_WAVES_HOST, "job lists are per wave");
static_assert(NET_KG_DWORDS == 9 * TAP_DWORDS && NET_KG_CHANNELS == 32, "host packing (engine.hip) and kernel agree");

__host__ __device__ constexpr int og_mask(int og) {
  return og == 0 ? 0x1FF : og == 1 ? 0x011 : og == 2 ? 0x00A : og == 3 ? 0x0A0 : og == 4 ? 0x144 :
         og == 5 ? 0x02F : og == 6 ? 0x1D0 : 0;
}

__device__ __forceinline__ int slot_addr(int cell, int pos, int s) {
  return ((cell * POS + pos) << 7) + (((s ^ (pos >> 1)) & 7) << 4);
}
__device__ __forceinline__ int strip_addr(int cell, int pos, int s) {
  return ((cell * POS + pos) << 5) + (((s ^ (pos >> 2)) & 1) << 4);
}

template <int I, int TAP>
struct TapMap {
  static constexpr int dy = TAP / 3 - 1, dx = TAP % 3 - 1;
  static constexpr int oy = I / 3 - dy, ox = I % 3 - dx;
  static constexpr bool valid = oy >= 0 && oy < 3 && ox >= 0 && ox < 3;
  static constexpr int o = valid ? oy * 3 + ox : 0;
};
template <int OMASK, int I, int TAP>
constexpr bool pair_used() { return TapMap<I, TAP>::valid && ((OMASK >> TapMap<I, TAP>::o) & 1); }
template <int OMASK, int I>
constexpr bool input_used() {
  return pair_used<OMASK, I, 0>() || pair_used<OMASK, I, 1>() || pair_used<OMASK, I, 2>() ||
         pair_used<OMASK, I, 3>() || pair_used<OMASK, I, 4>() || pair_used<OMASK, I, 5>() ||
         pair_used<OMASK, I, 6>() || pair_used<OMASK, I, 7>() || pair_used<OMASK, I, 8>();
}

template <int OMASK, int I>
constexpr int first_use() {
  return pair_used<OMASK, I, 0>() ? 0 : pair_used<OMASK, I, 1>() ? 1 : pair_used<OMASK, I, 2>() ? 2 :
         pair_used<OMASK, I, 3>() ? 3 : pair_used<OMASK, I, 4>() ? 4 : pair_used<OMASK, I, 5>() ? 5 :
         pair_used<OMASK, I, 6>() ? 6 : pair_used<OMASK, I, 7>() ? 7 : 8;
}
template <int OMASK, int I>
constexpr int last_use() {
  return pair_used<OMASK, I, 8>() ? 8 : pair_used<OMASK, I, 7>() ? 7 : pair_used<OMASK, I, 6>() ? 6 :
         pair_used<OMASK, I, 5>() ? 5 : pair_used<OMASK, I, 4>() ? 4 : pair_used<OMASK, I, 3>() ? 3 :
         pair_used<OMASK, I, 2>() ? 2 : pair_used<OMASK, I, 1>() ? 1 : 0;
}
constexpr int REFILL_AHEAD = 3;
template <int OMASK, int I>
constexpr int refill_step() {
  constexpr int earliest = last_use<OMASK, I>();
  constexpr int wanted = 9 + first_use<OMASK, I>() - REFILL_AHEAD;
  return wanted > earliest ? wanted : earliest;
}

struct Pieces {
  u32x4 p[3];
};
struct FragS {
  Pieces rb[W_RING];
};

__device__ __forceinline__ uint32_t trunc_bf16(float x) { return __builtin_bit_cast(uint32_t, x) & 0xFFFF0000u; }
__device__ __forceinline__ uint32_t pack_hi16(float x0, float x1) {
  return __builtin_amdgcn_perm(__builtin_bit_cast(uint32_t, x1), __builtin_bit_cast(uint32_t, x0), 0x07060302u);
}
__device__ __forceinline__ void split_pair(float x0, float x1, uint32_t& p0, uint32_t& p1, uint32_t& p2) {
  p0 = pack_hi16(x0, x1);
  const float r0 = x0 - __builtin_bit_cast(float, trunc_bf16(x0));
  const float r1 = x1 - __builtin_bit_cast(float, trunc_bf16(x1));
  p1 = pack_hi16(r0, r1);
  const float s0 = r0 - __builtin_bit_cast(float, trunc_bf16(r0));
  const float s1 = r1 - __builtin_bit_cast(float, trunc_bf16(r1));
  p2 = pack_hi16(s0, s1);
}
__device__ __forceinline__ float bf16_lo(uint32_t w) { return __builtin_bit_cast(float, w << 16); }
__device__ __forceinline__ float bf16_hi(uint32_t w) { return __builtin_bit_cast(float, w & 0xFFFF0000u); }

__device__ __forceinline__ f32x4 mfma_bf16(const u32x4& w, const u32x4& x, const f32x4& c) {
  return __builtin_amdgcn_mfma_f32_16x16x32_bf16(__builtin_bit_cast(bf16x8, w), __builtin_bit_cast(bf16x8, x), c, 0, 0, 0);
}
template <int OMASK, int I, int TAP>
__device__ __forceinline__ void pair_mfma(f32x4 (&acc)[CELLS], const Pieces (&x)[CELLS], const Pieces& w) {
  if constexpr (pair_used<OMASK, I, TAP>()) {
    constexpr int o = TapMap<I, TAP>::o;
    acc[o] = mfma_bf16(w.p[1], x[I].p[1], acc[o]);
    acc[o] = mfma_bf16(w.p[0], x[I].p[2], acc[o]);
    acc[o] = mfma_bf16(w.p[2], x[I].p[0], acc[o]);
    acc[o] = mfma_bf16(w.p[0], x[I].p[1], acc[o]);
    acc[o] = mfma_bf16(w.p[1], x[I].p[0], acc[o]);
    acc[o] = mfma_bf16(w.p[0], x[I].p[0], acc[o]);
    __builtin_amdgcn_sched_barrier(0);
  }
}
template <int OMASK, int TAP>
__device__ __forceinline__ void tap_mfma(f32x4 (&acc)[CELLS], const Pieces (&x)[CELLS], const Pieces& w) {
  pair_mfma<OMASK, 0, TAP>(acc, x, w); pair_mfma<OMASK, 1, TAP>(acc, x, w); pair_mfma<OMASK, 2, TAP>(acc, x, w);
  pair_mfma<OMASK, 3, TAP>(acc, x, w); pair_mfma<OMASK, 4, TAP>(acc, x, w); pair_mfma<OMASK, 5, TAP>(acc, x, w);
  pair_mfma<OMASK, 6, TAP>(acc, x, w); pair_mfma<OMASK, 7, TAP>(acc, x, w); pair_mfma<OMASK, 8, TAP>(acc, x, w);
}

template <int OMASK, int I>
__device__ __forceinline__ void load_cell(Pieces (&x)[CELLS], const unsigned char* __restrict__ src, int a0) {
#ifdef NZ_ABLATE_A
  if constexpr (input_used<OMASK, I>()) { const uint32_t v = 0x3C003C00u + a0 + I; x[I].p[0] = x[I].p[1] = x[I].p[2] = u32x4{v, v, v, v}; asm volatile("" :: "v"(src)); }
#else
  if constexpr (input_used<OMASK, I>()) {
#pragma unroll
    for (int piece = 0; piece < 3; ++piece)
      x[I].p[piece] = *reinterpret_cast<const u32x4*>(src + piece * PIECE_BYTES + I * (POS * 128) + a0);
  }
#endif
}
template <int OMASK>
__device__ __forceinline__ void load_cells(Pieces (&x)[CELLS], const unsigned char* __restrict__ src, int a0) {
  load_cell<OMASK, 0>(x, src, a0); load_cell<OMASK, 1>(x, src, a0); load_cell<OMASK, 2>(x, src, a0);
  load_cell<OMASK, 3>(x, src, a0); load_cell<OMASK, 4>(x, src, a0); load_cell<OMASK, 5>(x, src, a0);
  load_cell<OMASK, 6>(x, src, a0); load_cell<OMASK, 7>(x, src, a0); load_cell<OMASK, 8>(x, src, a0);
}
template <int OMASK, int I>
__device__ __forceinline__ void load_cell_split(Pieces (&x)[CELLS], const unsigned char* base, unsigned sh) {
  if constexpr (input_used<OMASK, I>()) {
#pragma unroll
    for (int piece = 0; piece < 3; ++piece)
      x[I].p[piece] = *reinterpret_cast<const u32x4*>(base + ((unsigned)(piece * STRIP_PIECE_BYTES + I * (POS * 32)) << sh));
  }
}
template <int OMASK>
__device__ __forceinline__ void load_cells_split(Pieces (&x)[CELLS], const unsigned char* __restrict__ src,
                                                 const unsigned char* __restrict__ strip, int pos, int quad) {
  const bool in_src = quad < 2;
  const unsigned char* base = in_src ? src + slot_addr(0, pos, 6 + quad) : strip + strip_addr(0, pos, quad - 2);
  const unsigned sh = in_src ? 2u : 0u;
  load_cell_split<OMASK, 0>(x, base, sh); load_cell_split<OMASK, 1>(x, base, sh); load_cell_split<OMASK, 2>(x, base, sh);
  load_cell_split<OMASK, 3>(x, base, sh); load_cell_split<OMASK, 4>(x, base, sh); load_cell_split<OMASK, 5>(x, base, sh);
  load_cell_split<OMASK, 6>(x, base, sh); load_cell_split<OMASK, 7>(x, base, sh); load_cell_split<OMASK, 8>(x, base, sh);
}
__device__ __forceinline__ void load_tap(Pieces& t, const float* __restrict__ w, int lane) {
#ifdef NZ_ABLATE_B
  const uint32_t v = 0x3C003C00u + lane;
  t.p[0] = t.p[1] = t.p[2] = u32x4{v, v, v, v};
  asm volatile("" :: "v"(w));
#else
  unsigned off = (unsigned)lane * 16u;
  asm volatile("" : "+v"(off));
  typedef const __attribute__((address_space(1))) u32x4* gptr;
  unsigned long long b = reinterpret_cast<unsigned long long>(w);
  asm volatile("" : "+s"(b));
  t.p[0] = *reinterpret_cast<gptr>(b + off);
  t.p[1] = *reinterpret_cast<gptr>(b + off + 1024);
  t.p[2] = *reinterpret_cast<gptr>(b + off + 2048);
#endif
}
__device__ __forceinline__ void load_b(FragS& f, const float* __restrict__ w, int lane) {
#pragma unroll
  for (int i = 0; i < W_RING; ++i) load_tap(f.rb[i], w + i * TAP_DWORDS, lane);
}
__device__ __forceinline__ void zero_b(FragS& f) {
#pragma unroll
  for (int t = 0; t < W_RING; ++t)
#pragma unroll
    for (int piece = 0; piece < 3; ++piece) f.rb[t].p[piece] = u32x4{0u, 0u, 0u, 0u};
}

template <int OMASK, int STEP>
__device__ __forceinline__ void refill(Pieces (&x)[CELLS], const unsigned char* __restrict__ src, int a1) {
  if constexpr (refill_step<OMASK, 0>() == STEP) load_cell<OMASK, 0>(x, src, a1);
  if constexpr (refill_step<OMASK, 1>() == STEP) load_cell<OMASK, 1>(x, src, a1);
  if constexpr (refill_step<OMASK, 2>() == STEP) load_cell<OMASK, 2>(x, src, a1);
  if constexpr (refill_step<OMASK, 3>() == STEP) load_cell<OMASK, 3>(x, src, a1);
  if constexpr (refill_step<OMASK, 4>() == STEP) load_cell<OMASK, 4>(x, src, a1);
  if constexpr (refill_step<OMASK, 5>() == STEP) load_cell<OMASK, 5>(x, src, a1);
  if constexpr (refill_step<OMASK, 6>() == STEP) load_cell<OMASK, 6>(x, src, a1);
  if constexpr (refill_step<OMASK, 7>() == STEP) load_cell<OMASK, 7>(x, src, a1);
  if constexpr (refill_step<OMASK, 8>() == STEP) load_cell<OMASK, 8>(x, src, a1);
}
template <int OMASK, int PART>
__device__ __forceinline__ void kgroup(f32x4 (&acc)[CELLS], Pieces (&x)[CELLS], FragS& f,
                                       const unsigned char* __restrict__ src, int a1,
                                       const float* __restrict__ wc, const float* __restrict__ wn, int lane) {
  constexpr bool A = PART == 1, B = PART == 2;
  if constexpr (B) refill<OMASK, 9>(x, src, a1);
  tap_mfma<OMASK, 0>(acc, x, f.rb[0]); load_tap(f.rb[0], wc + 3 * TAP_DWORDS, lane);
  if constexpr (A) refill<OMASK, 0>(x, src, a1);
  if constexpr (B) refill<OMASK, 10>(x, src, a1);
  tap_mfma<OMASK, 1>(acc, x, f.rb[1]); load_tap(f.rb[1], wc + 4 * TAP_DWORDS, lane);
  if constexpr (A) refill<OMASK, 1>(x, src, a1);
  if constexpr (B) refill<OMASK, 11>(x, src, a1);
  tap_mfma<OMASK, 2>(acc, x, f.rb[2]); load_tap(f.rb[2], wc + 5 * TAP_DWORDS, lane);
  if constexpr (A) refill<OMASK, 2>(x, src, a1);
  if constexpr (B) refill<OMASK, 12>(x, src, a1);
  tap_mfma<OMASK, 3>(acc, x, f.rb[0]); load_tap(f.rb[0], wc + 6 * TAP_DWORDS, lane);
  if constexpr (A) refill<OMASK, 3>(x, src, a1);
  if constexpr (B) refill<OMASK, 13>(x, src, a1);
  tap_mfma<OMASK, 4>(acc, x, f.rb[1]); load_tap(f.rb[1], wc + 7 * TAP_DWORDS, lane);
  if constexpr (A) refill<OMASK, 4>(x, src, a1);
  if constexpr (B) refill<OMASK, 14>(x, src, a1);
  tap_mfma<OMASK, 5>(acc, x, f.rb[2]); load_tap(f.rb[2], wc + 8 * TAP_DWORDS, lane);
  if constexpr (A) refill<OMASK, 5>(x, src, a1);
  if constexpr (B) refill<OMASK, 15>(x, src, a1);
  tap_mfma<OMASK, 6>(acc, x, f.rb[0]); load_tap(f.rb[0], wn + 0 * TAP_DWORDS, lane);
  if constexpr (A) refill<OMASK, 6>(x, src, a1);
  if constexpr (B) refill<OMASK, 16>(x, src, a1);
  tap_mfma<OMASK, 7>(acc, x, f.rb[1]); load_tap(f.rb[1], wn + 1 * TAP_DWORDS, lane);
  if constexpr (A) refill<OMASK, 7>(x, src, a1);
  if constexpr (B) refill<OMASK, 17>(x, src, a1);
  tap_mfma<OMASK, 8>(acc, x, f.rb[2]); load_tap(f.rb[2], wn + 2 * TAP_DWORDS, lane);
  if constexpr (A) refill<OMASK, 8>(x, src, a1);
}
template <int OMASK, int KG>
__device__ __forceinline__ void job_kloop(f32x4 (&acc)[CELLS], FragS& f, const unsigned char* __restrict__ src,
                                          const unsigned char* __restrict__ strip, int sslot,
                                          const float* __restrict__ w, const float* __restrict__ w_after, int lane) {
  const int pos = lane & 15, quad = lane >> 4;
  Pieces x[CELLS];
  if (KG == 1 && sslot == NET_SSLOT_SPLIT) load_cells_split<OMASK>(x, src, strip, pos, quad);
  else load_cells<OMASK>(x, src, slot_addr(0, pos, sslot + quad));
  if constexpr (KG == 2) {
    const int a1 = slot_addr(0, pos, sslot + 4 + quad);
    kgroup<OMASK, 1>(acc, x, f, src, a1, w, w + NET_KG_DWORDS, lane);
    kgroup<OMASK, 2>(acc, x, f, src, a1, w + NET_KG_DWORDS, w_after, lane);
  } else {
    kgroup<OMASK, 0>(acc, x, f, src, 0, w, w_after, lane);
  }
}

__device__ __forceinline__ float tanh_fast(float x) { return 1.0f - 2.0f / (__expf(2.0f * x) + 1.0f); }

template <int OMASK, int TAP, int I>
__device__ __forceinline__ void mfma_extra_pair(f32x4 (&acc)[CELLS], const float (&ax)[CELLS], const float (&bx)[9]) {
  if constexpr (pair_used<OMASK, I, TAP>()) {
    constexpr int o = TapMap<I, TAP>::o;
    acc[o] = __builtin_amdgcn_mfma_f32_16x16x4f32(bx[TAP], ax[I], acc[o], 0, 0, 0);
  }
}
template <int OMASK, int TAP>
__device__ __forceinline__ void mfma_extra_tap(f32x4 (&acc)[CELLS], const float (&ax)[CELLS], const float (&bx)[9]) {
  mfma_extra_pair<OMASK, TAP, 0>(acc, ax, bx); mfma_extra_pair<OMASK, TAP, 1>(acc, ax, bx);
  mfma_extra_pair<OMASK, TAP, 2>(acc, ax, bx); mfma_extra_pair<OMASK, TAP, 3>(acc, ax, bx);
  mfma_extra_pair<OMASK, TAP, 4>(acc, ax, bx); mfma_extra_pair<OMASK, TAP, 5>(acc, ax, bx);
  mfma_extra_pair<OMASK, TAP, 6>(acc, ax, bx); mfma_extra_pair<OMASK, TAP, 7>(acc, ax, bx);
  mfma_extra_pair<OMASK, TAP, 8>(acc, ax, bx);
}
template <int OMASK>
__device__ __forceinline__ void extra_planes(f32x4 (&acc)[CELLS], const float* __restrict__ wx,
                                             const float* __restrict__ inp, int lane) {
  float ax[CELLS], bx[9];
  const __attribute__((address_space(1))) float* wxg = (const __attribute__((address_space(1))) float*)wx;
  const __attribute__((address_space(3))) float* inl = (const __attribute__((address_space(3))) float*)inp;
#pragma unroll
  for (int t = 0; t < 9; ++t) bx[t] = wxg[t * 64 + lane];
#pragma unroll
  for (int i = 0; i < CELLS; ++i) ax[i] = inl[(i * POS + (lane & 15)) * 4 + (lane >> 4)];
  mfma_extra_tap<OMASK, 0>(acc, ax, bx); mfma_extra_tap<OMASK, 1>(acc, ax, bx); mfma_extra_tap<OMASK, 2>(acc, ax, bx);
  mfma_extra_tap<OMASK, 3>(acc, ax, bx); mfma_extra_tap<OMASK, 4>(acc, ax, bx); mfma_extra_tap<OMASK, 5>(acc, ax, bx);
  mfma_extra_tap<OMASK, 6>(acc, ax, bx); mfma_extra_tap<OMASK, 7>(acc, ax, bx); mfma_extra_tap<OMASK, 8>(acc, ax, bx);
}

template <int OMASK, int ACT, bool RES, bool STRIP = false>
__device__ __forceinline__ void epilogue_lds(const f32x4 (&acc)[CELLS], unsigned char* __restrict__ dst,
                                             const unsigned char* res, int lane, int nt) {
  const int pos = lane & 15, quad = lane >> 4;
  constexpr int PB = STRIP ? STRIP_PIECE_BYTES : PIECE_BYTES, CB = STRIP ? POS * 32 : POS * 128;
  const int off = (STRIP ? strip_addr(0, pos, quad >> 1) : slot_addr(0, pos, nt * 2 + (quad >> 1))) + (quad & 1) * 8;
#ifdef NZ_ABLATE_EPI
  {
    float t = 0.f;
#pragma unroll
    for (int o = 0; o < CELLS; ++o) if ((OMASK >> o) & 1) t += acc[o][0] + acc[o][1] + acc[o][2] + acc[o][3];
    *reinterpret_cast<float*>(dst + off) = t;
    return;
  }
#endif
  u32x2 q[CELLS][3];
  if constexpr (RES) {
#pragma unroll
    for (int o = 0; o < CELLS; ++o)
#pragma unroll
      for (int piece = 0; piece < 3; ++piece)
        if ((OMASK >> o) & 1) q[o][piece] = *reinterpret_cast<const u32x2*>(res + piece * PIECE_BYTES + o * (POS * 128) + off);
  }
#pragma unroll
  for (int o = 0; o < CELLS; ++o) {
    if (!((OMASK >> o) & 1)) continue;
    f32x4 v = acc[o];
    if constexpr (RES) {
      v[0] += (bf16_lo(q[o][0][0]) + bf16_lo(q[o][1][0])) + bf16_lo(q[o][2][0]);
      v[1] += (bf16_hi(q[o][0][0]) + bf16_hi(q[o][1][0])) + bf16_hi(q[o][2][0]);
      v[2] += (bf16_lo(q[o][0][1]) + bf16_lo(q[o][1][1])) + bf16_lo(q[o][2][1]);
      v[3] += (bf16_hi(q[o][0][1]) + bf16_hi(q[o][1][1])) + bf16_hi(q[o][2][1]);
    }
#pragma unroll
    for (int r = 0; r < 4; ++r) {
      float x = v[r];
      if constexpr (ACT == 1) x = fmaxf(x, 0.0f);
      if constexpr (ACT == 2) x = tanh_fast(x);
      if constexpr (ACT == 3) x = x > 0.0f ? x : expm1f(x);
      v[r] = x;
    }
    uint32_t a0, a1, a2, b0, b1, b2;
    split_pair(v[0], v[1], a0, a1, a2);
    split_pair(v[2], v[3], b0, b1, b2);
    *reinterpret_cast<u32x2*>(dst + 0 * PB + o * CB + off) = u32x2{a0, b0};
    *reinterpret_cast<u32x2*>(dst + 1 * PB + o * CB + off) = u32x2{a1, b1};
    *reinterpret_cast<u32x2*>(dst + 2 * PB + o * CB + off) = u32x2{a2, b2};
  }
}
template <int OMASK>
__device__ __forceinline__ void epilogue(const f32x4 (&acc)[CELLS], const NetJob& job, unsigned char* __restrict__ lds,
                                         unsigned char* __restrict__ strip, int lane, int policy_channels, int n_valid,
                                         float* logits, float* vcells) {
  if (job.dst == NET_DST_STRIP) {
    epilogue_lds<OMASK, 1, false, true>(acc, strip, nullptr, lane, 0);
  } else if (job.dst < NET_BUFFERS) {
    unsigned char* dst = lds + job.dst * ACT_BYTES;
    if (job.res >= 0) {
      epilogue_lds<OMASK, 1, true>(acc, dst, lds + job.res * ACT_BYTES, lane, job.dtile);
    } else if (job.act == 1) {
      epilogue_lds<OMASK, 1, false>(acc, dst, nullptr, lane, job.dtile);
    } else if (job.act == 2) {
      epilogue_lds<OMASK, 2, false>(acc, dst, nullptr, lane, job.dtile);
    } else if (job.act == 3) {
      epilogue_lds<OMASK, 3, false>(acc, dst, nullptr, lane, job.dtile);
    } else {
      epilogue_lds<OMASK, 0, false>(acc, dst, nullptr, lane, job.dtile);
    }
  } else if (job.dst == NET_DST_POLICY) {
    int l2 = lane;
    asm volatile("" : "+v"(l2));
    const int pos = l2 & 15, quad = l2 >> 4;
    if (pos < n_valid) {
#pragma unroll
      for (int r = 0; r < 4; ++r) {
        const int cout = job.nt * 16 + quad * 4 + r;
        if (cout < policy_channels) {
#pragma unroll
          for (int o = 0; o < CELLS; ++o)
            if ((OMASK >> o) & 1) logits[((size_t)pos * policy_channels + cout) * CELLS + o] = acc[o][r];
        }
      }
    }
  } else {
    int l2 = lane;
    asm volatile("" : "+v"(l2));
    const int pos = l2 & 15, quad = l2 >> 4;
    if (job.nt == 0 && quad == 0) {
#pragma unroll
      for (int o = 0; o < CELLS; ++o)
        if ((OMASK >> o) & 1) vcells[o * POS + pos] = acc[o][0];
    }
  }
}

template <int OMASK, typename Stamp, typename Fetch>
__device__ __forceinline__ void run_job(const NetJob& job, FragS& f, const float* __restrict__ W,
                                        const float* w_after, unsigned char* __restrict__ lds,
                                        unsigned char* __restrict__ strip,
                                        const float* __restrict__ inp, int lane, int policy_channels, int n_valid,
                                        float* logits, float* value, Stamp&& stamp, Fetch&& fetch_next) {
  asm volatile("" : "+v"(lane));
  f32x4 acc[CELLS];
#pragma unroll
  for (int o = 0; o < CELLS; ++o) acc[o] = f32x4{0.f, 0.f, 0.f, 0.f};
  if (job.kgroups == 2) job_kloop<OMASK, 2>(acc, f, lds + job.src * ACT_BYTES, strip, job.sslot, W + job.w_off, w_after, lane);
  else if (job.kgroups == 1) job_kloop<OMASK, 1>(acc, f, lds + job.src * ACT_BYTES, strip, job.sslot, W + job.w_off, w_after, lane);
  stamp(0);
  if (job.extra) extra_planes<OMASK>(acc, W + job.wx_off, inp, lane);
  stamp(1);
  fetch_next();
  epilogue<OMASK>(acc, job, lds, strip, lane, policy_channels, n_valid, logits, value);
  stamp(2);
}

template <bool STAMPS = false>
__device__ __forceinline__ void net_tile(const NetProgram* __restrict__ prog, const float* __restrict__ W,
                                         float* __restrict__ lds_f, const float* __restrict__ inp,
                                         int policy_channels, int n_valid, float* logits, float* value,
                                         unsigned long long* stamps = nullptr) {
  unsigned char* __restrict__ lds = reinterpret_cast<unsigned char*>(lds_f);
  float* const vcells = lds_f + NET_BUFFERS * ACT_FLOATS + INP_FLOATS;
  unsigned char* const strip = reinterpret_cast<unsigned char*>(vcells + VAL_FLOATS);
  int tid = threadIdx.x;
  asm volatile("" : "+v"(tid));
  const int lane = tid & 63;
  const int wave = __builtin_amdgcn_readfirstlane(tid >> 6);
  const NetJob* __restrict__ jobs = prog->jobs[wave];
  const int n_jobs = __builtin_amdgcn_readfirstlane(prog->n_jobs[wave]);
  const int first_w = __builtin_amdgcn_readfirstlane(prog->first_w_off[wave]);

  FragS f;
  zero_b(f);
  if (first_w >= 0) load_b(f, W + first_w, lane);

  unsigned long long tk[4] = {0, 0, 0, 0}, ts = 0;
#ifdef NZ_STAGE_STAMPS
  unsigned long long pk[3] = {0, 0, 0}, st_rec[24][3];
  int n_st = 0;
#endif
  auto stamp = [&](int slot) {
    if constexpr (STAMPS) {
      const unsigned long long now = __builtin_amdgcn_s_memtime();
      tk[slot] += now - ts;
      ts = now;
    }
  };
  if constexpr (STAMPS) ts = __builtin_amdgcn_s_memtime();

  static_assert(sizeof(NetJob) == 24, "six dwords");
  int vzero;
  asm volatile("v_mov_b32 %0, 0" : "=v"(vzero));
  const __attribute__((address_space(1))) uint32_t* jw =
      (const __attribute__((address_space(1))) uint32_t*)reinterpret_cast<const uint32_t*>(jobs) + vzero;
  uint32_t nw[6];
#pragma unroll
  for (int i = 0; i < 6; ++i) nw[i] = jw[i];
  for (int j = 0; j < n_jobs; ++j) {
    NetJob job;
    {
      uint32_t cw[6];
#pragma unroll
      for (int i = 0; i < 6; ++i) cw[i] = (uint32_t)__builtin_amdgcn_readfirstlane((int)nw[i]);
      __builtin_memcpy(&job, cw, sizeof(job));
    }
    __builtin_amdgcn_s_waitcnt(0x0F70);
    auto fetch_next = [&]() {
      if (j + 1 < n_jobs) {
#pragma unroll
        for (int i = 0; i < 6; ++i) nw[i] = jw[(j + 1) * 6 + i];
      }
    };
    if (job.og == OG_NONE) fetch_next();
    if (job.og != OG_NONE) {
      const float* w_after = W + (job.next_w_off >= 0 ? job.next_w_off : 0);
      switch (job.og) {
        case 1: run_job<og_mask(1)>(job, f, W, w_after, lds, strip, inp, lane, policy_channels, n_valid, logits, vcells, stamp, fetch_next); break;
        case 2: run_job<og_mask(2)>(job, f, W, w_after, lds, strip, inp, lane, policy_channels, n_valid, logits, vcells, stamp, fetch_next); break;
        case 3: run_job<og_mask(3)>(job, f, W, w_after, lds, strip, inp, lane, policy_channels, n_valid, logits, vcells, stamp, fetch_next); break;
        case 4: run_job<og_mask(4)>(job, f, W, w_after, lds, strip, inp, lane, policy_channels, n_valid, logits, vcells, stamp, fetch_next); break;
        case 5: run_job<og_mask(5)>(job, f, W, w_after, lds, strip, inp, lane, policy_channels, n_valid, logits, vcells, stamp, fetch_next); break;
        default: run_job<og_mask(6)>(job, f, W, w_after, lds, strip, inp, lane, policy_channels, n_valid, logits, vcells, stamp, fetch_next); break;
      }
    }
    stamp(2);
    if (job.stage_end) __syncthreads();
    stamp(3);
#ifdef NZ_STAGE_STAMPS
    if constexpr (STAMPS) {
      if (job.stage_end && blockIdx.x == 0 && (tid == 0 || tid == 256) && n_st < 24) {
        st_rec[n_st][0] = tk[0] + tk[1] - pk[0]; st_rec[n_st][1] = tk[2] - pk[1]; st_rec[n_st][2] = tk[3] - pk[2];
        ++n_st;
        pk[0] = tk[0] + tk[1]; pk[1] = tk[2]; pk[2] = tk[3];
      }
    }
#endif
  }
  if (tid < POS && tid < n_valid) {
    float sum = 0.0f;
#pragma unroll
    for (int o = 0; o < CELLS; ++o) sum += vcells[o * POS + tid];
    value[tid] = tanh_fast(sum / 9.0f);
  }
  __syncthreads();
  if constexpr (STAMPS) {
    if (tid == 0)
      for (int i = 0; i < 4; ++i) stamps[i] = tk[i];
#ifdef NZ_STAGE_STAMPS
    if (blockIdx.x == 0 && (tid == 0 || tid == 256))
      for (int i = 0; i < n_st; ++i)
        printf("wave %d stage %d: k %llu epi %llu bar %llu\n", wave, i, st_rec[i][0], st_rec[i][1], st_rec[i][2]);
#endif
  }
}

}
```

Measured before the change: 118,300 games/s.

## Interleave conv epilogue of early-finished cells into the K-loop for eligible jobs

Adds a progressive epilogue path. For output-cell groups whose cells have no remaining taps late in the K loop, activation, residual reads and LDS stores for those cells are scheduled inside the K-loop slots instead of after it. The host compiler marks a job progressive only when its destination buffer is not read by any job in the same stage, so writing early stays safe. The goal is to hide epilogue latency behind the MFMA/K-loop work. In exchange it adds template complexity, register pressure from the in-flight epilogue state, and more code variants. The host job-program builder is also refactored and exported for inspection.

```diff
diff --git a/include/nuzero_amd.h b/include/nuzero_amd.h
--- a/include/nuzero_amd.h
+++ b/include/nuzero_amd.h
@@ -114,6 +114,11 @@
 
 nz_status nz_engine_net_flops(const nz_engine* e, double* flops_host);
 nz_status nz_engine_net_matrix_flops(const nz_engine* e, double* bf16_flops_host, double* f32_flops_host);
+
+#define NZ_NET_JOB_FIELDS 13
+nz_status nz_net_program(const nz_net_desc* net, int32_t recurrent_iterations, int32_t* jobs, int32_t max_jobs,
+                         int32_t* n_jobs);
+int32_t nz_net_final_tap(int32_t cell);
 
 nz_status nz_net_forward(nz_engine* e, const float* states_dev, int32_t batch, float* logits_dev,
                          float* value_dev, float* probs_dev, void* stream);
diff --git a/nuzero_amd/_lib.py b/nuzero_amd/_lib.py
--- a/nuzero_amd/_lib.py
+++ b/nuzero_amd/_lib.py
@@ -14,6 +14,7 @@
 NZ_ARCH_RECURRENT, NZ_ARCH_RESNET, NZ_ARCH_CONVNET = 0, 1, 2
 NZ_LOSS_CE, NZ_LOSS_KLD, NZ_LOSS_MSE = 0, 1, 2
 NZ_LOSS_SE, NZ_LOSS_AE = 0, 1
+NZ_NET_JOB_FIELDS = 13
 
 
 class SearchCfg(Structure):
@@ -95,6 +96,8 @@
     "nz_engine_counters_n": (c_int32, [c_void_p, POINTER(c_int64), c_int32, c_void_p]),
     "nz_engine_net_flops": (c_int32, [c_void_p, POINTER(c_double)]),
     "nz_engine_net_matrix_flops": (c_int32, [c_void_p, POINTER(c_double), POINTER(c_double)]),
+    "nz_net_program": (c_int32, [POINTER(NetDesc), c_int32, c_void_p, c_int32, POINTER(c_int32)]),
+    "nz_net_final_tap": (c_int32, [c_int32]),
     "nz_net_forward": (c_int32, [c_void_p, c_void_p, c_int32, c_void_p, c_void_p, c_void_p, c_void_p]),
     "nz_net_forward_stamps": (c_int32, [c_void_p, c_void_p, c_int32, c_void_p, c_void_p, POINTER(c_double)]),
     "nz_engine_profile": (c_int32, [c_void_p, c_int32]),
diff --git a/nuzero_amd/csrc/engine.h b/nuzero_amd/csrc/engine.h
--- a/nuzero_amd/csrc/engine.h
+++ b/nuzero_amd/csrc/engine.h
@@ -119,9 +119,19 @@
   int8_t src, dst;
   int8_t res;
   int8_t act;
-  int8_t stage_end;
+  int8_t flags;
   int8_t dtile;
 };
+constexpr int NET_JOB_STAGE_END = 1;
+constexpr int NET_JOB_PROGRESSIVE = 2;
+__host__ __device__ constexpr int og_mask(int og) {
+  return og == 0 ? 0x1FF : og == 1 ? 0x011 : og == 2 ? 0x00A : og == 3 ? 0x0A0 : og == 4 ? 0x144 :
+         og == 5 ? 0x02F : og == 6 ? 0x1D0 : 0;
+}
+__host__ __device__ constexpr int net_final_tap(int o) {
+  return 3 * ((o / 3 < 2 ? 1 : 0) + 1) + ((o % 3 < 2 ? 1 : 0) + 1);
+}
+__host__ __device__ constexpr bool net_og_progressive(int cells) { return cells == 0x1D0 || cells == 0x0A0 || cells == 0x144; }
 constexpr int NET_WAVES_HOST = 8;
 constexpr int NET_MAX_JOBS = 192;
 constexpr int OG_NONE = 7;
diff --git a/nuzero_amd/csrc/engine.hip b/nuzero_amd/csrc/engine.hip
--- a/nuzero_amd/csrc/engine.hip
+++ b/nuzero_amd/csrc/engine.hip
@@ -243,6 +243,17 @@
     if (u.job.dst == NET_DST_STRIP && (u.job.dtile != 0 || u.job.act != 1 || u.job.res >= 0)) return false;
     if (u.job.sslot == NET_SSLOT_SPLIT && u.job.kgroups != 1) return false;
   }
+  unsigned read_areas = 0;
+  for (const Unit& u : units) {
+    if (u.job.kgroups > 0) read_areas |= 1u << u.job.src;
+    if (u.job.sslot == NET_SSLOT_SPLIT) read_areas |= 1u << NET_ACT_BUFFERS;
+  }
+  for (Unit& u : units) {
+    NetJob& j = u.job;
+    const bool form = j.dst >= 0 && j.dst < NET_ACT_BUFFERS && j.kgroups >= 1 && !j.extra && j.sslot != NET_SSLOT_SPLIT &&
+                      net_og_progressive(og_mask(j.og)) && (j.res >= 0 ? j.act == 1 : (j.act == 1 || j.act == 2));
+    if (form && !((read_areas >> j.dst) & 1)) j.flags |= NET_JOB_PROGRESSIVE;
+  }
   int load[NET_WAVES_HOST];
   std::vector<int> who(units.size());
   deal(units, load, who.data());
@@ -260,9 +271,102 @@
       j.og = OG_NONE;
       pg.jobs[w][pg.n_jobs[w]++] = j;
     }
-    pg.jobs[w][pg.n_jobs[w] - 1].stage_end = 1;
+    pg.jobs[w][pg.n_jobs[w] - 1].flags |= NET_JOB_STAGE_END;
   }
   return true;
+}
+
+struct ConvShape { int cout, cin, k; };
+struct NetLayout {
+  bool recall;
+  int iterations, trunk_tensors, trunk_k;
+  std::vector<ConvShape> shapes;
+  int cin_main(int i, int in_planes) const {
+    const bool with_planes = (i == 0) || (recall && i == 1);
+    return with_planes ? shapes[i].cin - in_planes : shapes[i].cin;
+  }
+};
+std::string text(const char* fmt, ...) {
+  char buf[256];
+  va_list ap;
+  va_start(ap, fmt);
+  vsnprintf(buf, sizeof(buf), fmt, ap);
+  va_end(ap);
+  return buf;
+}
+std::string net_layout(const nz_net_desc* net, int recurrent_iterations, NetLayout& L) {
+  if (net->hex) return "hexagonal convolutions are built for nz_boardnet_* only";
+  if (net->in_channels != 2 || net->policy_channels != 1) return "Tic-Tac-Toe nets take 2 input planes and 1 policy plane";
+  if (net->width <= 0 || net->width > 64 || net->width % 4 != 0) return "width must be a multiple of 4 in (0, 64]";
+  if (net->num_blocks < 0 || recurrent_iterations < 0) return "negative block/iteration count";
+  const int arch = net->arch;
+  if (arch != NZ_ARCH_RECURRENT && arch != NZ_ARCH_RESNET && arch != NZ_ARCH_CONVNET) return text("unknown architecture %d", arch);
+  L.trunk_k = arch == NZ_ARCH_CONVNET ? net->kernel_size : 3;
+  if (L.trunk_k != 1 && L.trunk_k != 3) return "ConvNet kernel_size must be 1 or 3";
+  L.recall = arch == NZ_ARCH_RECURRENT && net->recall;
+  L.iterations = arch == NZ_ARCH_RECURRENT ? recurrent_iterations : 1;
+  L.trunk_tensors = arch == NZ_ARCH_CONVNET ? 1 + net->num_blocks : 1 + (L.recall ? 1 : 0) + 2 * net->num_blocks;
+  if (1 + L.iterations * (L.trunk_tensors - 1) + 24 > NET_MAX_JOBS)
+    return text("too many layers for one fused launch (%d iterations)", recurrent_iterations);
+  const int W = net->width, IN = net->in_channels;
+  std::vector<ConvShape>& shapes = L.shapes;
+  shapes.clear();
+  shapes.push_back({W, IN, L.trunk_k});
+  if (L.recall) shapes.push_back({W, W + IN, 3});
+  for (int i = (int)shapes.size(); i < L.trunk_tensors; ++i) shapes.push_back({W, W, L.trunk_k});
+  for (int i = 0; i < 2; ++i)
+    shapes.push_back({head_channel(W, net->policy_channels, 2, i + 1), head_channel(W, net->policy_channels, 2, i), 3});
+  for (int i = 0; i < 4; ++i) shapes.push_back({head_channel(W, 1, 4, i + 1), head_channel(W, 1, 4, i), 3});
+  return "";
+}
+std::string compile_net(const nz_net_desc* net, const NetLayout& L, const std::vector<PackedConv>& convs, NetProgram& pg,
+                        double& flops) {
+  const std::vector<ConvShape>& shapes = L.shapes;
+  const int arch = net->arch, trunk_tensors = L.trunk_tensors, iterations = L.iterations;
+  const bool recall = L.recall;
+  flops = 0.0;
+  memset(&pg, 0, sizeof(pg));
+  bool ok = true;
+  int cur = 0;
+  auto stage = [&](std::vector<StageConv> convs_in_stage) {
+    for (const StageConv& sc : convs_in_stage)
+      flops += 2.0 * shapes[sc.tensor].cout * shapes[sc.tensor].cin * (shapes[sc.tensor].k == 3 ? 49.0 : 9.0);
+    ok = ok && add_stage(pg, convs, convs_in_stage);
+  };
+  if (arch == NZ_ARCH_CONVNET) {
+    stage({{0, 0, cur, -1, 3, true}});
+    for (int i = 1; i < trunk_tensors; ++i) { stage({{i, cur, cur ^ 1, -1, 3, true}}); cur ^= 1; }
+  } else {
+    stage({{0, 0, cur, -1, 1, true}});
+    const int first_block = recall ? 2 : 1;
+    for (int it = 0; it < iterations; ++it) {
+      if (recall) { stage({{1, cur, cur ^ 1, -1, 0, true}}); cur ^= 1; }
+      for (int b = 0; b < net->num_blocks; ++b) {
+        stage({{first_block + 2 * b, cur, cur ^ 1, -1, 1, true}});
+        stage({{first_block + 2 * b + 1, cur ^ 1, cur, cur, 1, true}});
+      }
+    }
+  }
+  const int ph = trunk_tensors, vh = ph + 2;
+  const int vact = net->value_activation == NZ_ACT_RELU ? 1 : 2;
+  const int side = cur ^ 1;
+  const int tv0 = convs[vh].ntiles, tp0 = convs[ph].ntiles;
+  if (tv0 + tp0 > 5 || (tv0 + tp0 == 5 && tv0 != 3)) return text("head layout: %d + %d tiles", tv0, tp0);
+  const int p1_sslot = tv0 + tp0 <= 4 ? 2 * tv0 : NET_SSLOT_SPLIT;
+  stage({{vh, cur, side, -1, vact, true, 0, 0}, {ph, cur, side, -1, 1, true, 0, tv0}});
+  stage({{vh + 1, side, cur, -1, vact, true}, {ph + 1, side, NET_DST_POLICY, -1, 0, true, p1_sslot, 0}});
+  stage({{vh + 2, cur, side, -1, vact, true}});
+  stage({{vh + 3, side, NET_DST_VALUE, -1, 0, true}});
+  if (!ok) return text("network too deep for one fused launch (%d iterations)", iterations);
+  for (int w = 0; w < NET_WAVES_HOST; ++w) {
+    int32_t next = -1;
+    for (int j = pg.n_jobs[w] - 1; j >= 0; --j) {
+      pg.jobs[w][j].next_w_off = next;
+      if (pg.jobs[w][j].og != OG_NONE && pg.jobs[w][j].kgroups > 0) next = pg.jobs[w][j].w_off;
+    }
+    pg.first_w_off[w] = next;
+  }
+  return "";
 }
 
 hipStream_t as_stream(void* s) { return static_cast<hipStream_t>(s); }
@@ -423,35 +527,13 @@
 nz_status nz_engine_set_weights(nz_engine* e, const nz_net_desc* net, const float* const* weights,
                                 int32_t n_tensors, int32_t recurrent_iterations) {
   if (!e || !net || !weights) return NZ_ERR_ARG;
-  if (net->hex) return fail(e, NZ_ERR_ARG, "hexagonal convolutions are built for nz_boardnet_* only");
-  if (net->in_channels != 2 || net->policy_channels != 1)
-    return fail(e, NZ_ERR_ARG, "Tic-Tac-Toe nets take 2 input planes and 1 policy plane");
-  if (net->width <= 0 || net->width > 64 || net->width % 4 != 0)
-    return fail(e, NZ_ERR_ARG, "width must be a multiple of 4 in (0, 64]");
-  if (net->num_blocks < 0 || recurrent_iterations < 0) return fail(e, NZ_ERR_ARG, "negative block/iteration count");
-  const int arch = net->arch;
-  if (arch != NZ_ARCH_RECURRENT && arch != NZ_ARCH_RESNET && arch != NZ_ARCH_CONVNET)
-    return fail(e, NZ_ERR_ARG, "unknown architecture %d", arch);
-  const int trunk_k = arch == NZ_ARCH_CONVNET ? net->kernel_size : 3;
-  if (trunk_k != 1 && trunk_k != 3) return fail(e, NZ_ERR_ARG, "ConvNet kernel_size must be 1 or 3");
-  const bool recall = arch == NZ_ARCH_RECURRENT && net->recall;
-  const int iterations = arch == NZ_ARCH_RECURRENT ? recurrent_iterations : 1;
-  const int trunk_tensors = arch == NZ_ARCH_CONVNET ? 1 + net->num_blocks : 1 + (recall ? 1 : 0) + 2 * net->num_blocks;
-  const int expect = trunk_tensors + 2 + 4;
+  NetLayout L;
+  const std::string bad = net_layout(net, recurrent_iterations, L);
+  if (!bad.empty()) return fail(e, NZ_ERR_ARG, "%s", bad.c_str());
+  const int expect = (int)L.shapes.size();
   if (n_tensors != expect) return fail(e, NZ_ERR_ARG, "expected %d weight tensors, got %d", expect, n_tensors);
-  if (1 + iterations * (trunk_tensors - 1) + 24 > NET_MAX_JOBS)
-    return fail(e, NZ_ERR_ARG, "too many layers for one fused launch (%d iterations)", recurrent_iterations);
-  NZ_HIP(e, hipSetDevice(e->device));
-
-  const int W = net->width, IN = net->in_channels;
-  struct Shape { int cout, cin, k; };
-  std::vector<Shape> shapes;
-  shapes.push_back({W, IN, trunk_k});
-  if (recall) shapes.push_back({W, W + IN, 3});
-  for (int i = (int)shapes.size(); i < trunk_tensors; ++i) shapes.push_back({W, W, trunk_k});
-  for (int i = 0; i < 2; ++i)
-    shapes.push_back({head_channel(W, net->policy_channels, 2, i + 1), head_channel(W, net->policy_channels, 2, i), 3});
-  for (int i = 0; i < 4; ++i) shapes.push_back({head_channel(W, 1, 4, i + 1), head_channel(W, 1, 4, i), 3});
+  NZ_HIP(e, hipSetDevice(e->device));
+  const std::vector<ConvShape>& shapes = L.shapes;
 
   std::vector<std::vector<float>> host(n_tensors);
   for (int i = 0; i < n_tensors; ++i) {
@@ -468,55 +550,14 @@
 
   std::vector<float> packed;
   std::vector<PackedConv> convs(n_tensors);
+  for (int i = 0; i < n_tensors; ++i) {
+    convs[i] = pack_conv(host[i].data(), shapes[i].cout, shapes[i].cin, L.cin_main(i, net->in_channels), packed);
+  }
+
+  NetProgram& pg = e->prog_host;
   double flops = 0.0;
-  for (int i = 0; i < n_tensors; ++i) {
-    const bool with_planes = (i == 0) || (recall && i == 1);
-    const int cin_main = with_planes ? shapes[i].cin - IN : shapes[i].cin;
-    convs[i] = pack_conv(host[i].data(), shapes[i].cout, shapes[i].cin, cin_main, packed);
-  }
-
-  NetProgram& pg = e->prog_host;
-  memset(&pg, 0, sizeof(pg));
-  bool ok = true;
-  int cur = 0;
-  auto stage = [&](std::vector<StageConv> convs_in_stage) {
-    for (const StageConv& sc : convs_in_stage)
-      flops += 2.0 * shapes[sc.tensor].cout * shapes[sc.tensor].cin * (shapes[sc.tensor].k == 3 ? 49.0 : 9.0);
-    ok = ok && add_stage(pg, convs, convs_in_stage);
-  };
-  if (arch == NZ_ARCH_CONVNET) {
-    stage({{0, 0, cur, -1, 3, true}});
-    for (int i = 1; i < trunk_tensors; ++i) { stage({{i, cur, cur ^ 1, -1, 3, true}}); cur ^= 1; }
-  } else {
-    stage({{0, 0, cur, -1, 1, true}});
-    const int first_block = recall ? 2 : 1;
-    for (int it = 0; it < iterations; ++it) {
-      if (recall) { stage({{1, cur, cur ^ 1, -1, 0, true}}); cur ^= 1; }
-      for (int b = 0; b < net->num_blocks; ++b) {
-        stage({{first_block + 2 * b, cur, cur ^ 1, -1, 1, true}});
-        stage({{first_block + 2 * b + 1, cur ^ 1, cur, cur, 1, true}});
-      }
-    }
-  }
-  const int ph = trunk_tensors, vh = ph + 2;
-  const int vact = net->value_activation == NZ_ACT_RELU ? 1 : 2;
-  const int side = cur ^ 1;
-  const int tv0 = convs[vh].ntiles, tp0 = convs[ph].ntiles;
-  if (tv0 + tp0 > 5 || (tv0 + tp0 == 5 && tv0 != 3)) return fail(e, NZ_ERR_ARG, "head layout: %d + %d tiles", tv0, tp0);
-  const int p1_sslot = tv0 + tp0 <= 4 ? 2 * tv0 : NET_SSLOT_SPLIT;
-  stage({{vh, cur, side, -1, vact, true, 0, 0}, {ph, cur, side, -1, 1, true, 0, tv0}});
-  stage({{vh + 1, side, cur, -1, vact, true}, {ph + 1, side, NET_DST_POLICY, -1, 0, true, p1_sslot, 0}});
-  stage({{vh + 2, cur, side, -1, vact, true}});
-  stage({{vh + 3, side, NET_DST_VALUE, -1, 0, true}});
-  if (!ok) return fail(e, NZ_ERR_ARG, "network too deep for one fused launch (%d iterations)", recurrent_iterations);
-  for (int w = 0; w < NET_WAVES_HOST; ++w) {
-    int32_t next = -1;
-    for (int j = pg.n_jobs[w] - 1; j >= 0; --j) {
-      pg.jobs[w][j].next_w_off = next;
-      if (pg.jobs[w][j].og != OG_NONE && pg.jobs[w][j].kgroups > 0) next = pg.jobs[w][j].w_off;
-    }
-    pg.first_w_off[w] = next;
-  }
+  const std::string deep = compile_net(net, L, convs, pg, flops);
+  if (!deep.empty()) return fail(e, NZ_ERR_ARG, "%s", deep.c_str());
   e->algorithmic_flops_per_position = flops;
   {
     double bf16 = 0.0, f32 = 0.0;
@@ -541,6 +582,51 @@
   e->tp.table = nullptr;
   return NZ_OK;
 }
+
+nz_status nz_net_program(const nz_net_desc* net, int32_t recurrent_iterations, int32_t* jobs, int32_t max_jobs,
+                         int32_t* n_jobs) {
+  if (!net || !n_jobs || (!jobs && max_jobs > 0)) return NZ_ERR_ARG;
+  NetLayout L;
+  std::string bad = net_layout(net, recurrent_iterations, L);
+  std::vector<float> packed;
+  std::vector<PackedConv> convs(L.shapes.size());
+  NetProgram* pg = new NetProgram;
+  if (bad.empty()) {
+    for (size_t i = 0; i < L.shapes.size(); ++i) {
+      const std::vector<float> zeros((size_t)L.shapes[i].cout * L.shapes[i].cin * 9, 0.f);
+      convs[i] = pack_conv(zeros.data(), L.shapes[i].cout, L.shapes[i].cin, L.cin_main((int)i, net->in_channels), packed);
+    }
+    double flops = 0.0;
+    bad = compile_net(net, L, convs, *pg, flops);
+  }
+  if (!bad.empty()) {
+    delete pg;
+    g_create_error = bad;
+    return NZ_ERR_ARG;
+  }
+  int32_t n = 0;
+  for (int w = 0; w < NET_WAVES_HOST; ++w) {
+    int stage = 0;
+    for (int j = 0; j < pg->n_jobs[w]; ++j) {
+      const NetJob& job = pg->jobs[w][j];
+      if (job.og != OG_NONE) {
+        if (n < max_jobs) {
+          const int32_t row[NZ_NET_JOB_FIELDS] = {w, stage, job.og, og_mask(job.og), job.kgroups, job.sslot, job.src, job.dst,
+                                                  job.res, job.act, job.dtile, job.extra,
+                                                  (job.flags & NET_JOB_PROGRESSIVE) ? 1 : 0};
+          memcpy(jobs + (size_t)n * NZ_NET_JOB_FIELDS, row, sizeof(row));
+        }
+        ++n;
+      }
+      if (job.flags & NET_JOB_STAGE_END) ++stage;
+    }
+  }
+  delete pg;
+  *n_jobs = n;
+  return NZ_OK;
+}
+
+int32_t nz_net_final_tap(int32_t cell) { return cell >= 0 && cell < 9 ? net_final_tap(cell) : -1; }
 
 nz_status nz_engine_set_table(nz_engine* e, const float* table, int32_t n_rows) {
   if (!e || !table) return NZ_ERR_ARG;
diff --git a/nuzero_amd/csrc/net_dev.hpp b/nuzero_amd/csrc/net_dev.hpp
--- a/nuzero_amd/csrc/net_dev.hpp
+++ b/nuzero_amd/csrc/net_dev.hpp
@@ -27,10 +27,6 @@
 static_assert(NET_WAVES == NET_WAVES_HOST, "job lists are per wave");
 static_assert(NET_KG_DWORDS == 9 * TAP_DWORDS && NET_KG_CHANNELS == 32, "host packing (engine.hip) and kernel agree");
 
-__host__ __device__ constexpr int og_mask(int og) {
-  return og == 0 ? 0x1FF : og == 1 ? 0x011 : og == 2 ? 0x00A : og == 3 ? 0x0A0 : og == 4 ? 0x144 :
-         og == 5 ? 0x02F : og == 6 ? 0x1D0 : 0;
-}
 
 __device__ __forceinline__ int slot_addr(int cell, int pos, int s) {
   return ((cell * POS + pos) << 7) + (((s ^ (pos >> 1)) & 7) << 4);
@@ -67,6 +63,37 @@
          pair_used<OMASK, I, 5>() ? 5 : pair_used<OMASK, I, 4>() ? 4 : pair_used<OMASK, I, 3>() ? 3 :
          pair_used<OMASK, I, 2>() ? 2 : pair_used<OMASK, I, 1>() ? 1 : 0;
 }
+template <int OMASK, int O>
+constexpr int final_tap() {
+  static_assert((OMASK >> O) & 1, "cell of the job's group");
+  return net_final_tap(O);
+}
+static_assert(net_final_tap(8) == 4 && net_final_tap(6) == 5 && net_final_tap(7) == 5 && net_final_tap(2) == 7 &&
+              net_final_tap(5) == 7 && net_final_tap(0) == 8 && net_final_tap(1) == 8 && net_final_tap(3) == 8 &&
+              net_final_tap(4) == 8, "tap = 3 (dy + 1) + (dx + 1), input cell = output cell + (dy, dx)");
+constexpr int pairs_before(int omask, int tap, int i) {
+  int n = 0;
+  for (int t = 0; t < 9; ++t)
+    for (int c = 0; c < CELLS; ++c) {
+      const int oy = c / 3 - (t / 3 - 1), ox = c % 3 - (t % 3 - 1);
+      const bool used = oy >= 0 && oy < 3 && ox >= 0 && ox < 3 && ((omask >> (oy * 3 + ox)) & 1);
+      if (used && (t < tap || (t == tap && c < i))) ++n;
+    }
+  return n;
+}
+static_assert(pairs_before(0x1FF, 9, 0) == 49 && pairs_before(0x02F, 9, 0) == 26 && pairs_before(0x1D0, 9, 0) == 23, "og_mask");
+constexpr int early_cell(int omask, int qi) {
+  for (int t = 0; t < 8; ++t)
+    for (int o = 0; o < CELLS; ++o)
+      if (((omask >> o) & 1) && net_final_tap(o) == t && qi-- == 0) return o;
+  return -1;
+}
+constexpr int early_cells(int omask) {
+  int n = 0;
+  while (early_cell(omask, n) >= 0) ++n;
+  return n;
+}
+
 constexpr int REFILL_AHEAD = 3;
 template <int OMASK, int I>
 constexpr int refill_step() {
@@ -101,24 +128,29 @@
 __device__ __forceinline__ f32x4 mfma_bf16(const u32x4& w, const u32x4& x, const f32x4& c) {
   return __builtin_amdgcn_mfma_f32_16x16x32_bf16(__builtin_bit_cast(bf16x8, w), __builtin_bit_cast(bf16x8, x), c, 0, 0, 0);
 }
-template <int OMASK, int I, int TAP>
-__device__ __forceinline__ void pair_mfma(f32x4 (&acc)[CELLS], const Pieces (&x)[CELLS], const Pieces& w) {
+struct NoEpi {
+  template <int G>
+  __device__ __forceinline__ void slot(const f32x4 (&)[CELLS]) {}
+};
+template <int OMASK, int I, int TAP, typename E>
+__device__ __forceinline__ void pair_mfma(f32x4 (&acc)[CELLS], const Pieces (&x)[CELLS], const Pieces& w, E& e) {
   if constexpr (pair_used<OMASK, I, TAP>()) {
     constexpr int o = TapMap<I, TAP>::o;
-    acc[o] = mfma_bf16(w.p[1], x[I].p[1], acc[o]);
-    acc[o] = mfma_bf16(w.p[0], x[I].p[2], acc[o]);
-    acc[o] = mfma_bf16(w.p[2], x[I].p[0], acc[o]);
-    acc[o] = mfma_bf16(w.p[0], x[I].p[1], acc[o]);
-    acc[o] = mfma_bf16(w.p[1], x[I].p[0], acc[o]);
-    acc[o] = mfma_bf16(w.p[0], x[I].p[0], acc[o]);
+    constexpr int g = 6 * pairs_before(OMASK, TAP, I);
+    acc[o] = mfma_bf16(w.p[1], x[I].p[1], acc[o]); e.template slot<g + 0>(acc);
+    acc[o] = mfma_bf16(w.p[0], x[I].p[2], acc[o]); e.template slot<g + 1>(acc);
+    acc[o] = mfma_bf16(w.p[2], x[I].p[0], acc[o]); e.template slot<g + 2>(acc);
+    acc[o] = mfma_bf16(w.p[0], x[I].p[1], acc[o]); e.template slot<g + 3>(acc);
+    acc[o] = mfma_bf16(w.p[1], x[I].p[0], acc[o]); e.template slot<g + 4>(acc);
+    acc[o] = mfma_bf16(w.p[0], x[I].p[0], acc[o]); e.template slot<g + 5>(acc);
     __builtin_amdgcn_sched_barrier(0);
   }
 }
-template <int OMASK, int TAP>
-__device__ __forceinline__ void tap_mfma(f32x4 (&acc)[CELLS], const Pieces (&x)[CELLS], const Pieces& w) {
-  pair_mfma<OMASK, 0, TAP>(acc, x, w); pair_mfma<OMASK, 1, TAP>(acc, x, w); pair_mfma<OMASK, 2, TAP>(acc, x, w);
-  pair_mfma<OMASK, 3, TAP>(acc, x, w); pair_mfma<OMASK, 4, TAP>(acc, x, w); pair_mfma<OMASK, 5, TAP>(acc, x, w);
-  pair_mfma<OMASK, 6, TAP>(acc, x, w); pair_mfma<OMASK, 7, TAP>(acc, x, w); pair_mfma<OMASK, 8, TAP>(acc, x, w);
+template <int OMASK, int TAP, typename E>
+__device__ __forceinline__ void tap_mfma(f32x4 (&acc)[CELLS], const Pieces (&x)[CELLS], const Pieces& w, E& e) {
+  pair_mfma<OMASK, 0, TAP>(acc, x, w, e); pair_mfma<OMASK, 1, TAP>(acc, x, w, e); pair_mfma<OMASK, 2, TAP>(acc, x, w, e);
+  pair_mfma<OMASK, 3, TAP>(acc, x, w, e); pair_mfma<OMASK, 4, TAP>(acc, x, w, e); pair_mfma<OMASK, 5, TAP>(acc, x, w, e);
+  pair_mfma<OMASK, 6, TAP>(acc, x, w, e); pair_mfma<OMASK, 7, TAP>(acc, x, w, e); pair_mfma<OMASK, 8, TAP>(acc, x, w, e);
 }
 
 template <int OMASK, int I>
@@ -196,53 +228,54 @@
   if constexpr (refill_step<OMASK, 7>() == STEP) load_cell<OMASK, 7>(x, src, a1);
   if constexpr (refill_step<OMASK, 8>() == STEP) load_cell<OMASK, 8>(x, src, a1);
 }
-template <int OMASK, int PART>
+template <int OMASK, int PART, typename E>
 __device__ __forceinline__ void kgroup(f32x4 (&acc)[CELLS], Pieces (&x)[CELLS], FragS& f,
                                        const unsigned char* __restrict__ src, int a1,
-                                       const float* __restrict__ wc, const float* __restrict__ wn, int lane) {
+                                       const float* __restrict__ wc, const float* __restrict__ wn, int lane, E& e) {
   constexpr bool A = PART == 1, B = PART == 2;
   if constexpr (B) refill<OMASK, 9>(x, src, a1);
-  tap_mfma<OMASK, 0>(acc, x, f.rb[0]); load_tap(f.rb[0], wc + 3 * TAP_DWORDS, lane);
+  tap_mfma<OMASK, 0>(acc, x, f.rb[0], e); load_tap(f.rb[0], wc + 3 * TAP_DWORDS, lane);
   if constexpr (A) refill<OMASK, 0>(x, src, a1);
   if constexpr (B) refill<OMASK, 10>(x, src, a1);
-  tap_mfma<OMASK, 1>(acc, x, f.rb[1]); load_tap(f.rb[1], wc + 4 * TAP_DWORDS, lane);
+  tap_mfma<OMASK, 1>(acc, x, f.rb[1], e); load_tap(f.rb[1], wc + 4 * TAP_DWORDS, lane);
   if constexpr (A) refill<OMASK, 1>(x, src, a1);
   if constexpr (B) refill<OMASK, 11>(x, src, a1);
-  tap_mfma<OMASK, 2>(acc, x, f.rb[2]); load_tap(f.rb[2], wc + 5 * TAP_DWORDS, lane);
+  tap_mfma<OMASK, 2>(acc, x, f.rb[2], e); load_tap(f.rb[2], wc + 5 * TAP_DWORDS, lane);
   if constexpr (A) refill<OMASK, 2>(x, src, a1);
   if constexpr (B) refill<OMASK, 12>(x, src, a1);
-  tap_mfma<OMASK, 3>(acc, x, f.rb[0]); load_tap(f.rb[0], wc + 6 * TAP_DWORDS, lane);
+  tap_mfma<OMASK, 3>(acc, x, f.rb[0], e); load_tap(f.rb[0], wc + 6 * TAP_DWORDS, lane);
   if constexpr (A) refill<OMASK, 3>(x, src, a1);
   if constexpr (B) refill<OMASK, 13>(x, src, a1);
-  tap_mfma<OMASK, 4>(acc, x, f.rb[1]); load_tap(f.rb[1], wc + 7 * TAP_DWORDS, lane);
+  tap_mfma<OMASK, 4>(acc, x, f.rb[1], e); load_tap(f.rb[1], wc + 7 * TAP_DWORDS, lane);
   if constexpr (A) refill<OMASK, 4>(x, src, a1);
   if constexpr (B) refill<OMASK, 14>(x, src, a1);
-  tap_mfma<OMASK, 5>(acc, x, f.rb[2]); load_tap(f.rb[2], wc + 8 * TAP_DWORDS, lane);
+  tap_mfma<OMASK, 5>(acc, x, f.rb[2], e); load_tap(f.rb[2], wc + 8 * TAP_DWORDS, lane);
   if constexpr (A) refill<OMASK, 5>(x, src, a1);
   if constexpr (B) refill<OMASK, 15>(x, src, a1);
-  tap_mfma<OMASK, 6>(acc, x, f.rb[0]); load_tap(f.rb[0], wn + 0 * TAP_DWORDS, lane);
+  tap_mfma<OMASK, 6>(acc, x, f.rb[0], e); load_tap(f.rb[0], wn + 0 * TAP_DWORDS, lane);
   if constexpr (A) refill<OMASK, 6>(x, src, a1);
   if constexpr (B) refill<OMASK, 16>(x, src, a1);
-  tap_mfma<OMASK, 7>(acc, x, f.rb[1]); load_tap(f.rb[1], wn + 1 * TAP_DWORDS, lane);
+  tap_mfma<OMASK, 7>(acc, x, f.rb[1], e); load_tap(f.rb[1], wn + 1 * TAP_DWORDS, lane);
   if constexpr (A) refill<OMASK, 7>(x, src, a1);
   if constexpr (B) refill<OMASK, 17>(x, src, a1);
-  tap_mfma<OMASK, 8>(acc, x, f.rb[2]); load_tap(f.rb[2], wn + 2 * TAP_DWORDS, lane);
+  tap_mfma<OMASK, 8>(acc, x, f.rb[2], e); load_tap(f.rb[2], wn + 2 * TAP_DWORDS, lane);
   if constexpr (A) refill<OMASK, 8>(x, src, a1);
 }
-template <int OMASK, int KG>
+template <int OMASK, int KG, typename E>
 __device__ __forceinline__ void job_kloop(f32x4 (&acc)[CELLS], FragS& f, const unsigned char* __restrict__ src,
                                           const unsigned char* __restrict__ strip, int sslot,
-                                          const float* __restrict__ w, const float* __restrict__ w_after, int lane) {
+                                          const float* __restrict__ w, const float* __restrict__ w_after, int lane, E& e) {
   const int pos = lane & 15, quad = lane >> 4;
   Pieces x[CELLS];
   if (KG == 1 && sslot == NET_SSLOT_SPLIT) load_cells_split<OMASK>(x, src, strip, pos, quad);
   else load_cells<OMASK>(x, src, slot_addr(0, pos, sslot + quad));
   if constexpr (KG == 2) {
     const int a1 = slot_addr(0, pos, sslot + 4 + quad);
-    kgroup<OMASK, 1>(acc, x, f, src, a1, w, w + NET_KG_DWORDS, lane);
-    kgroup<OMASK, 2>(acc, x, f, src, a1, w + NET_KG_DWORDS, w_after, lane);
+    NoEpi none;
+    kgroup<OMASK, 1>(acc, x, f, src, a1, w, w + NET_KG_DWORDS, lane, none);
+    kgroup<OMASK, 2>(acc, x, f, src, a1, w + NET_KG_DWORDS, w_after, lane, e);
   } else {
-    kgroup<OMASK, 0>(acc, x, f, src, 0, w, w_after, lane);
+    kgroup<OMASK, 0>(acc, x, f, src, 0, w, w_after, lane, e);
   }
 }
 
@@ -278,12 +311,109 @@
   mfma_extra_tap<OMASK, 6>(acc, ax, bx); mfma_extra_tap<OMASK, 7>(acc, ax, bx); mfma_extra_tap<OMASK, 8>(acc, ax, bx);
 }
 
+constexpr int early_begin(int omask, int ns, int qi) {
+  int b = 0, end = 0;
+  for (int q = 0; q <= qi; ++q) {
+    const int start = 6 * pairs_before(omask, net_final_tap(early_cell(omask, q)) + 1, 0);
+    b = start > end ? start : end;
+    end = b + ns;
+  }
+  return b;
+}
+template <int ACT, bool RES>
+constexpr int epi_steps() { return (RES ? 8 : 1) + (ACT >= 2 ? 4 : 1) + 7; }
+struct EpiRegs {
+  f32x4 v;
+  u32x2 q[3];
+  float c[3];
+  float r[4];
+};
+template <int ACT>
+__device__ __forceinline__ float epi_act(float x) {
+  if constexpr (ACT == 1) x = fmaxf(x, 0.0f);
+  if constexpr (ACT == 2) x = tanh_fast(x);
+  if constexpr (ACT == 3) x = x > 0.0f ? x : expm1f(x);
+  return x;
+}
+__device__ __forceinline__ float epi_rem(float x) { return x - __builtin_bit_cast(float, trunc_bf16(x)); }
+template <bool STRIP>
+__device__ __forceinline__ int epi_off(int lane, int nt) {
+  const int pos = lane & 15, quad = lane >> 4;
+  return (STRIP ? strip_addr(0, pos, quad >> 1) : slot_addr(0, pos, nt * 2 + (quad >> 1))) + (quad & 1) * 8;
+}
+template <int O>
+__device__ __forceinline__ void epi_read_res(u32x2 (&q)[3], const unsigned char* res, int off) {
+#pragma unroll
+  for (int piece = 0; piece < 3; ++piece)
+    q[piece] = *reinterpret_cast<const u32x2*>(res + piece * PIECE_BYTES + O * (POS * 128) + off);
+}
+template <int ACT, bool RES, bool STRIP, int O, int K>
+__device__ __forceinline__ void epi_step(EpiRegs& s, const f32x4& a, unsigned char* __restrict__ dst, int off) {
+  constexpr int PB = STRIP ? STRIP_PIECE_BYTES : PIECE_BYTES, CB = STRIP ? POS * 32 : POS * 128;
+  constexpr int NR = RES ? 8 : 1, NA = ACT >= 2 ? 4 : 1;
+  static_assert(K >= 0 && K < NR + NA + 7, "step of the sequence");
+  if constexpr (K < NR) {
+    if constexpr (RES) {
+      constexpr int r = K >> 1;
+      if constexpr ((K & 1) == 0) {
+#pragma unroll
+        for (int piece = 0; piece < 3; ++piece) s.c[piece] = (r & 1) ? bf16_hi(s.q[piece][r >> 1]) : bf16_lo(s.q[piece][r >> 1]);
+      } else {
+        s.v[r] = a[r] + ((s.c[0] + s.c[1]) + s.c[2]);
+      }
+    }
+  } else if constexpr (K < NR + NA) {
+    if constexpr (NA == 4) {
+      constexpr int r = K - NR;
+      s.v[r] = epi_act<ACT>(RES ? s.v[r] : a[r]);
+    } else {
+#pragma unroll
+      for (int r = 0; r < 4; ++r) s.v[r] = epi_act<ACT>(RES ? s.v[r] : a[r]);
+    }
+  } else {
+    constexpr int P = K - NR - NA;
+    unsigned char* const d = dst + O * CB + off;
+    if constexpr (P == 0) *reinterpret_cast<u32x2*>(d + 0 * PB) = u32x2{pack_hi16(s.v[0], s.v[1]), pack_hi16(s.v[2], s.v[3])};
+    if constexpr (P == 1) { s.r[0] = epi_rem(s.v[0]); s.r[1] = epi_rem(s.v[1]); }
+    if constexpr (P == 2) { s.r[2] = epi_rem(s.v[2]); s.r[3] = epi_rem(s.v[3]); }
+    if constexpr (P == 3) *reinterpret_cast<u32x2*>(d + 1 * PB) = u32x2{pack_hi16(s.r[0], s.r[1]), pack_hi16(s.r[2], s.r[3])};
+    if constexpr (P == 4) { s.r[0] = epi_rem(s.r[0]); s.r[1] = epi_rem(s.r[1]); }
+    if constexpr (P == 5) { s.r[2] = epi_rem(s.r[2]); s.r[3] = epi_rem(s.r[3]); }
+    if constexpr (P == 6) *reinterpret_cast<u32x2*>(d + 2 * PB) = u32x2{pack_hi16(s.r[0], s.r[1]), pack_hi16(s.r[2], s.r[3])};
+  }
+}
+template <int ACT, bool RES, bool STRIP, int O, int K0>
+__device__ __forceinline__ void epi_steps_from(EpiRegs& s, const f32x4& a, unsigned char* __restrict__ dst, int off) {
+  if constexpr (K0 < epi_steps<ACT, RES>()) {
+    epi_step<ACT, RES, STRIP, O, K0>(s, a, dst, off);
+    epi_steps_from<ACT, RES, STRIP, O, K0 + 1>(s, a, dst, off);
+  }
+}
+template <int O, int ACT, bool RES, bool STRIP>
+__device__ __forceinline__ void epilogue_cell(const f32x4& a, const u32x2 (&q)[3], unsigned char* __restrict__ dst, int off) {
+  EpiRegs s;
+  if constexpr (RES) { s.q[0] = q[0]; s.q[1] = q[1]; s.q[2] = q[2]; }
+  epi_steps_from<ACT, RES, STRIP, O, 0>(s, a, dst, off);
+}
+template <int CMASK, int ACT, bool RES, bool STRIP, int O = 0>
+__device__ __forceinline__ void epilogue_cells(const f32x4 (&acc)[CELLS], const u32x2 (&q)[CELLS][3],
+                                               unsigned char* __restrict__ dst, int off) {
+  if constexpr (O < CELLS) {
+    if constexpr ((CMASK >> O) & 1) epilogue_cell<O, ACT, RES, STRIP>(acc[O], q[O], dst, off);
+    epilogue_cells<CMASK, ACT, RES, STRIP, O + 1>(acc, q, dst, off);
+  }
+}
+template <int CMASK, int O = 0>
+__device__ __forceinline__ void epi_read_cells(u32x2 (&q)[CELLS][3], const unsigned char* res, int off) {
+  if constexpr (O < CELLS) {
+    if constexpr ((CMASK >> O) & 1) epi_read_res<O>(q[O], res, off);
+    epi_read_cells<CMASK, O + 1>(q, res, off);
+  }
+}
 template <int OMASK, int ACT, bool RES, bool STRIP = false>
 __device__ __forceinline__ void epilogue_lds(const f32x4 (&acc)[CELLS], unsigned char* __restrict__ dst,
                                              const unsigned char* res, int lane, int nt) {
-  const int pos = lane & 15, quad = lane >> 4;
-  constexpr int PB = STRIP ? STRIP_PIECE_BYTES : PIECE_BYTES, CB = STRIP ? POS * 32 : POS * 128;
-  const int off = (STRIP ? strip_addr(0, pos, quad >> 1) : slot_addr(0, pos, nt * 2 + (quad >> 1))) + (quad & 1) * 8;
+  const int off = epi_off<STRIP>(lane, nt);
 #ifdef NZ_ABLATE_EPI
   {
     float t = 0.f;
@@ -294,39 +424,67 @@
   }
 #endif
   u32x2 q[CELLS][3];
-  if constexpr (RES) {
-#pragma unroll
-    for (int o = 0; o < CELLS; ++o)
-#pragma unroll
-      for (int piece = 0; piece < 3; ++piece)
-        if ((OMASK >> o) & 1) q[o][piece] = *reinterpret_cast<const u32x2*>(res + piece * PIECE_BYTES + o * (POS * 128) + off);
-  }
-#pragma unroll
-  for (int o = 0; o < CELLS; ++o) {
-    if (!((OMASK >> o) & 1)) continue;
-    f32x4 v = acc[o];
-    if constexpr (RES) {
-      v[0] += (bf16_lo(q[o][0][0]) + bf16_lo(q[o][1][0])) + bf16_lo(q[o][2][0]);
-      v[1] += (bf16_hi(q[o][0][0]) + bf16_hi(q[o][1][0])) + bf16_hi(q[o][2][0]);
-      v[2] += (bf16_lo(q[o][0][1]) + bf16_lo(q[o][1][1])) + bf16_lo(q[o][2][1]);
-      v[3] += (bf16_hi(q[o][0][1]) + bf16_hi(q[o][1][1])) + bf16_hi(q[o][2][1]);
-    }
-#pragma unroll
-    for (int r = 0; r < 4; ++r) {
-      float x = v[r];
-      if constexpr (ACT == 1) x = fmaxf(x, 0.0f);
-      if constexpr (ACT == 2) x = tanh_fast(x);
-      if constexpr (ACT == 3) x = x > 0.0f ? x : expm1f(x);
-      v[r] = x;
-    }
-    uint32_t a0, a1, a2, b0, b1, b2;
-    split_pair(v[0], v[1], a0, a1, a2);
-    split_pair(v[2], v[3], b0, b1, b2);
-    *reinterpret_cast<u32x2*>(dst + 0 * PB + o * CB + off) = u32x2{a0, b0};
-    *reinterpret_cast<u32x2*>(dst + 1 * PB + o * CB + off) = u32x2{a1, b1};
-    *reinterpret_cast<u32x2*>(dst + 2 * PB + o * CB + off) = u32x2{a2, b2};
-  }
-}
+  if constexpr (RES) epi_read_cells<OMASK>(q, res, off);
+  epilogue_cells<OMASK, ACT, RES, STRIP>(acc, q, dst, off);
+}
+
+template <int OMASK, int ACT, bool RES>
+struct ProgEpi {
+  static constexpr int NS = epi_steps<ACT, RES>(), NQ = early_cells(OMASK), SLOTS = 6 * pairs_before(OMASK, 9, 0);
+  static constexpr int READ_AHEAD = 6;
+  static constexpr int LATE = OMASK & 0x01B;
+  static_assert(NQ >= 1 && NQ <= 3, "groups with early cells");
+  static constexpr int B0 = early_begin(OMASK, NS, 0), B1 = NQ > 1 ? early_begin(OMASK, NS, 1) : 0, B2 = NQ > 2 ? early_begin(OMASK, NS, 2) : 0;
+  static constexpr int C0 = early_cell(OMASK, 0), C1 = early_cell(OMASK, 1), C2 = early_cell(OMASK, 2);
+  static constexpr int FIRST = RES ? B0 - READ_AHEAD : B0;
+  static_assert(FIRST >= 0 && FIRST < SLOTS && (!RES || READ_AHEAD <= NS - 8), "reads land inside the K group, behind the residual steps");
+  static constexpr int cell(int qi) { return qi == 0 ? C0 : qi == 1 ? C1 : C2; }
+  static constexpr int begin(int qi) { return qi == 0 ? B0 : qi == 1 ? B1 : B2; }
+  static constexpr int read_slot(int qi) { return begin(qi) - READ_AHEAD; }
+
+  EpiRegs s;
+  unsigned char* dst;
+  const unsigned char* res;
+  int lane, nt, off;
+
+  template <int QI, int G>
+  __device__ __forceinline__ void slot_of(const f32x4 (&acc)[CELLS]) {
+    if constexpr (QI < NQ) {
+      if constexpr (RES && G == read_slot(QI)) epi_read_res<cell(QI)>(s.q, res, off);
+      if constexpr (G >= begin(QI) && G < begin(QI) + NS) epi_step<ACT, RES, false, cell(QI), G - begin(QI)>(s, acc[cell(QI)], dst, off);
+    }
+  }
+  template <int QI, int G>
+  static constexpr bool busy() {
+    if constexpr (QI < NQ) return (RES && G == read_slot(QI)) || (G >= begin(QI) && G < begin(QI) + NS);
+    return false;
+  }
+  template <int G>
+  __device__ __forceinline__ void slot(const f32x4 (&acc)[CELLS]) {
+    if constexpr (busy<0, G>() || busy<1, G>() || busy<2, G>()) {
+      __builtin_amdgcn_sched_barrier(0);
+      if constexpr (G == FIRST) off = epi_off<false>(lane, nt);
+      slot_of<0, G>(acc); slot_of<1, G>(acc); slot_of<2, G>(acc);
+      __builtin_amdgcn_sched_barrier(0);
+    }
+  }
+  template <int QI>
+  __device__ __forceinline__ void finish_early(const f32x4 (&acc)[CELLS]) {
+    if constexpr (QI < NQ) {
+      if constexpr (RES && read_slot(QI) >= SLOTS) epi_read_res<cell(QI)>(s.q, res, off);
+      constexpr int done = SLOTS - begin(QI);
+      epi_steps_from<ACT, RES, false, cell(QI), (done > 0 ? done : 0)>(s, acc[cell(QI)], dst, off);
+      finish_early<QI + 1>(acc);
+    }
+  }
+  __device__ __forceinline__ void finish(const f32x4 (&acc)[CELLS]) {
+    u32x2 q[CELLS][3];
+    if constexpr (RES) epi_read_cells<LATE>(q, res, off);
+    finish_early<0>(acc);
+    epilogue_cells<LATE, ACT, RES, false>(acc, q, dst, off);
+  }
+};
+
 template <int OMASK>
 __device__ __forceinline__ void epilogue(const f32x4 (&acc)[CELLS], const NetJob& job, unsigned char* __restrict__ lds,
                                          unsigned char* __restrict__ strip, int lane, int policy_channels, int n_valid,
@@ -374,23 +532,63 @@
 }
 
 template <int OMASK, typename Stamp, typename Fetch>
-__device__ __forceinline__ void run_job(const NetJob& job, FragS& f, const float* __restrict__ W,
-                                        const float* w_after, unsigned char* __restrict__ lds,
-                                        unsigned char* __restrict__ strip,
-                                        const float* __restrict__ inp, int lane, int policy_channels, int n_valid,
-                                        float* logits, float* value, Stamp&& stamp, Fetch&& fetch_next) {
+__device__ __forceinline__ void run_job_plain(const NetJob& job, FragS& f, const float* __restrict__ W,
+                                              const float* w_after, unsigned char* __restrict__ lds,
+                                              unsigned char* __restrict__ strip,
+                                              const float* __restrict__ inp, int lane, int policy_channels, int n_valid,
+                                              float* logits, float* value, Stamp&& stamp, Fetch&& fetch_next) {
   asm volatile("" : "+v"(lane));
   f32x4 acc[CELLS];
 #pragma unroll
   for (int o = 0; o < CELLS; ++o) acc[o] = f32x4{0.f, 0.f, 0.f, 0.f};
-  if (job.kgroups == 2) job_kloop<OMASK, 2>(acc, f, lds + job.src * ACT_BYTES, strip, job.sslot, W + job.w_off, w_after, lane);
-  else if (job.kgroups == 1) job_kloop<OMASK, 1>(acc, f, lds + job.src * ACT_BYTES, strip, job.sslot, W + job.w_off, w_after, lane);
+  NoEpi none;
+  if (job.kgroups == 2) job_kloop<OMASK, 2>(acc, f, lds + job.src * ACT_BYTES, strip, job.sslot, W + job.w_off, w_after, lane, none);
+  else if (job.kgroups == 1) job_kloop<OMASK, 1>(acc, f, lds + job.src * ACT_BYTES, strip, job.sslot, W + job.w_off, w_after, lane, none);
   stamp(0);
   if (job.extra) extra_planes<OMASK>(acc, W + job.wx_off, inp, lane);
   stamp(1);
   fetch_next();
   epilogue<OMASK>(acc, job, lds, strip, lane, policy_channels, n_valid, logits, value);
   stamp(2);
+}
+template <int OMASK, int ACT, bool RES, typename Stamp, typename Fetch>
+__device__ __forceinline__ void run_job_prog(const NetJob& job, FragS& f, const float* __restrict__ W,
+                                             const float* w_after, unsigned char* __restrict__ lds,
+                                             unsigned char* __restrict__ strip, int lane, Stamp&& stamp, Fetch&& fetch_next) {
+  asm volatile("" : "+v"(lane));
+  f32x4 acc[CELLS];
+#pragma unroll
+  for (int o = 0; o < CELLS; ++o) acc[o] = f32x4{0.f, 0.f, 0.f, 0.f};
+  ProgEpi<OMASK, ACT, RES> e;
+  e.dst = lds + job.dst * ACT_BYTES;
+  e.res = lds + (RES ? job.res : 0) * ACT_BYTES;
+  e.lane = lane;
+  e.nt = job.dtile;
+  if (job.kgroups == 2) job_kloop<OMASK, 2>(acc, f, lds + job.src * ACT_BYTES, strip, job.sslot, W + job.w_off, w_after, lane, e);
+  else job_kloop<OMASK, 1>(acc, f, lds + job.src * ACT_BYTES, strip, job.sslot, W + job.w_off, w_after, lane, e);
+  stamp(0);
+  stamp(1);
+  fetch_next();
+  e.finish(acc);
+  stamp(2);
+}
+template <int OMASK, typename Stamp, typename Fetch>
+__device__ __forceinline__ void run_job(const NetJob& job, FragS& f, const float* __restrict__ W,
+                                        const float* w_after, unsigned char* __restrict__ lds,
+                                        unsigned char* __restrict__ strip,
+                                        const float* __restrict__ inp, int lane, int policy_channels, int n_valid,
+                                        float* logits, float* value, Stamp&& stamp, Fetch&& fetch_next) {
+#ifndef NZ_ABLATE_EPI
+  if constexpr (net_og_progressive(OMASK)) {
+    if (job.flags & NET_JOB_PROGRESSIVE) {
+      if (job.res >= 0) run_job_prog<OMASK, 1, true>(job, f, W, w_after, lds, strip, lane, stamp, fetch_next);
+      else if (job.act == 2) run_job_prog<OMASK, 2, false>(job, f, W, w_after, lds, strip, lane, stamp, fetch_next);
+      else run_job_prog<OMASK, 1, false>(job, f, W, w_after, lds, strip, lane, stamp, fetch_next);
+      return;
+    }
+  }
+#endif
+  run_job_plain<OMASK>(job, f, W, w_after, lds, strip, inp, lane, policy_channels, n_valid, logits, value, stamp, fetch_next);
 }
 
 template <bool STAMPS = false>
@@ -463,11 +661,11 @@
       }
     }
     stamp(2);
-    if (job.stage_end) __syncthreads();
+    if (job.flags & NET_JOB_STAGE_END) __syncthreads();
     stamp(3);
 #ifdef NZ_STAGE_STAMPS
     if constexpr (STAMPS) {
-      if (job.stage_end && blockIdx.x == 0 && (tid == 0 || tid == 256) && n_st < 24) {
+      if ((job.flags & NET_JOB_STAGE_END) && blockIdx.x == 0 && (tid == 0 || tid == 256) && n_st < 24) {
         st_rec[n_st][0] = tk[0] + tk[1] - pk[0]; st_rec[n_st][1] = tk[2] - pk[1]; st_rec[n_st][2] = tk[3] - pk[2];
         ++n_st;
         pk[0] = tk[0] + tk[1]; pk[1] = tk[2]; pk[2] = tk[3];
```

After: 120,200 games/s, median of 6. +1.6%, better.
